# laboshinl/loam_velodyne

Hardware: AMD Instinct MI355X
Metric: sweeps/sec (64-ring, 1M-pt map): feature extraction + odometry + scan-to-map registration (higher is better)
Workload: dtype f32

## Files before the change

### include/loamx.h

```cpp
#ifndef LOAMX_H
#define LOAMX_H

#include <stddef.h>
#include <stdint.h>

#ifdef __cplusplus
extern "C" {
#endif

#define LOAMX_OK 0
#define LOAMX_SKIPPED 1
#define LOAMX_E_INVALID (-1)
#define LOAMX_E_CAPACITY (-2)
#define LOAMX_E_HIP (-3)
#define LOAMX_E_NOGPU (-4)
#define LOAMX_E_UNSUPPORTED (-5)

typedef struct loamx_cloud {
  void* data;
  uint32_t count;
  uint32_t stride;
  uint32_t intensity_offset;
  uint32_t reserved;
} loamx_cloud;

const char* loamx_last_error(void);
int loamx_device_count(void);
#define LOAMX_ABI_VERSION 6
int loamx_abi_version(void);
const char* loamx_build_info(void);
void* loamx_host_alloc(size_t bytes);
void loamx_host_free(void* p);

typedef struct loamx_scanreg loamx_scanreg;

typedef struct loamx_scanreg_config {
  float scan_period;
  int n_feature_regions;
  int curvature_region;
  int max_corner_sharp;
  int max_surface_flat;
  float less_flat_filter_size;
  float surface_curvature_threshold;
  int device;
  int max_corner_less_sharp;
  int imu_history_size;
} loamx_scanreg_config;

void loamx_scanreg_default_config(loamx_scanreg_config* cfg);
loamx_scanreg* loamx_scanreg_create(const loamx_scanreg_config* cfg);
void loamx_scanreg_destroy(loamx_scanreg* h);
int loamx_scanreg_configure(loamx_scanreg* h, const loamx_scanreg_config* cfg);
int loamx_scanreg_process(loamx_scanreg* h, const loamx_cloud* cloud, const uint32_t* ring_size, uint32_t n_rings,
                          loamx_cloud* sharp, loamx_cloud* less_sharp, loamx_cloud* flat, loamx_cloud* less_flat);

typedef struct loamx_multiscan_mapper {
  float lower_bound_deg;
  float upper_bound_deg;
  uint32_t n_scan_rings;
} loamx_multiscan_mapper;
int loamx_multiscan_mapper_preset(const char* sensor , loamx_multiscan_mapper* out);
int loamx_scanreg_process_raw(loamx_scanreg* h, const loamx_multiscan_mapper* mapper, const void* raw_xyz, uint32_t count,
                              uint32_t stride, loamx_cloud* full, uint32_t* ring_size, loamx_cloud* sharp, loamx_cloud* less_sharp,
                              loamx_cloud* flat, loamx_cloud* less_flat);

int loamx_scanreg_update_imu(loamx_scanreg* h, double stamp_sec, float roll, float pitch, float yaw, const float acc_xyz[3]);
int loamx_scanreg_set_time(loamx_scanreg* h, double scan_time_sec);
int loamx_scanreg_get_imu_trans(loamx_scanreg* h, float imu_trans[12]);

typedef struct loamx_odom loamx_odom;

typedef struct loamx_odom_config {
  float scan_period;
  int max_iterations;
  float delta_t_abort;
  float delta_r_abort;
  int device;
} loamx_odom_config;

void loamx_odom_default_config(loamx_odom_config* cfg);
loamx_odom* loamx_odom_create(const loamx_odom_config* cfg);
void loamx_odom_destroy(loamx_odom* h);
int loamx_odom_update_imu(loamx_odom* h, const float imu_trans[12]);
int loamx_odom_process(loamx_odom* h, const loamx_cloud* sharp, const loamx_cloud* less_sharp, const loamx_cloud* flat,
                       const loamx_cloud* less_flat);
int loamx_odom_get_transform(loamx_odom* h, float transform[6]);
int loamx_odom_get_transform_sum(loamx_odom* h, float transform_sum[6]);
int loamx_odom_set_transform(loamx_odom* h, const float transform[6]);
int loamx_odom_set_transform_sum(loamx_odom* h, const float transform_sum[6]);
int loamx_odom_get_last_clouds(loamx_odom* h, loamx_cloud* last_corner, loamx_cloud* last_surf);
int loamx_odom_transform_to_end(loamx_odom* h, loamx_cloud* cloud);
int loamx_odom_get_stats(loamx_odom* h, int stats[4]);

int loamx_scanreg_process_linked(loamx_scanreg* h, const loamx_cloud* cloud, const uint32_t* ring_size, uint32_t n_rings);
int loamx_odom_process_linked(loamx_odom* h, loamx_scanreg* sr);
int loamx_odom_link_wait(loamx_odom* h);

typedef struct loamx_map loamx_map;

typedef struct loamx_map_config {
  float scan_period;
  int max_iterations;
  float delta_t_abort;
  float delta_r_abort;
  float corner_filter_size;
  float surf_filter_size;
  float map_filter_size;
  int device;
} loamx_map_config;

void loamx_map_default_config(loamx_map_config* cfg);
loamx_map* loamx_map_create(const loamx_map_config* cfg);
void loamx_map_destroy(loamx_map* h);
int loamx_map_update_odometry(loamx_map* h, const float transform_sum[6]);
int loamx_map_process(loamx_map* h, const loamx_cloud* corner_last, const loamx_cloud* surf_last, loamx_cloud* full_res);
int loamx_map_process_linked(loamx_map* h, loamx_odom* od, loamx_cloud* full_res_registered);
int loamx_map_get_speculation(loamx_map* h, uint64_t counts[2]);
int loamx_map_insert(loamx_map* h, const loamx_cloud* corner_last, const loamx_cloud* surf_last, const float pose6[6]);
int loamx_map_get_transform(loamx_map* h, int which, float transform[6]);
int loamx_map_set_transform(loamx_map* h, int which, const float transform[6]);
int loamx_map_update_imu(loamx_map* h, double stamp_sec, float roll, float pitch);
int loamx_map_set_time(loamx_map* h, double laser_odometry_time_sec);
int loamx_map_has_fresh_map(loamx_map* h);
int loamx_map_get_surround(loamx_map* h, loamx_cloud* out);
int loamx_map_load_cubes(loamx_map* h, const loamx_cloud* corner, const loamx_cloud* surf);
int loamx_map_get_cubes(loamx_map* h, int which, loamx_cloud* out);
int loamx_map_save_snapshot(loamx_map* h, const char* path);
int loamx_map_load_snapshot(loamx_map* h, const char* path);
int loamx_map_set_timing(loamx_map* h, int on);
int loamx_map_get_timing(loamx_map* h, float ms[4], uint64_t counts[4]);
int loamx_map_get_stats(loamx_map* h, int stats[8]);

typedef struct loamx_tm loamx_tm;
loamx_tm* loamx_tm_create(void);
void loamx_tm_destroy(loamx_tm* h);
int loamx_tm_update_odometry(loamx_tm* h, const float transform_sum[6]);
int loamx_tm_update_mapping_transform(loamx_tm* h, const float aft_mapped[6], const float bef_mapped[6]);
int loamx_tm_associate_to_map(loamx_tm* h);
int loamx_tm_get_mapped(loamx_tm* h, float transform_mapped[6]);
int loamx_wire_pose_to_quat(const float rot_xyz[3], double quat_xyzw[4]);
int loamx_wire_quat_to_pose(const double quat_xyzw[4], float rot_xyz[3]);

typedef struct loamx_batch loamx_batch;

loamx_batch* loamx_batch_create(const loamx_map_config* cfg, uint32_t max_sweeps);
void loamx_batch_destroy(loamx_batch* h);
int loamx_batch_set_frozen(loamx_batch* h, const loamx_cloud* corner_map, const loamx_cloud* surf_map);
int loamx_batch_set_frozen_device(loamx_batch* h, const void* d_corner_xyzi, uint32_t n_corner, const void* d_surf_xyzi,
                                  uint32_t n_surf);
int loamx_batch_stage_frozen_device(loamx_batch* h, const void* d_corner_xyzi, uint32_t n_corner, const void* d_surf_xyzi,
                                    uint32_t n_surf, void* wait_event );
int loamx_batch_stage_frozen(loamx_batch* h, const loamx_cloud* corner_map, const loamx_cloud* surf_map);
int loamx_batch_swap_frozen(loamx_batch* h);
int loamx_batch_upload(loamx_batch* h, uint32_t n_sweeps, const loamx_cloud* corner_last, const loamx_cloud* surf_last,
                       const loamx_cloud* full_res, const float* guess6);
int loamx_batch_run(loamx_batch* h);
int loamx_batch_run_async(loamx_batch* h);
int loamx_batch_sync(loamx_batch* h);
int loamx_batch_download(loamx_batch* h, float* poses6, int* stats4);
int loamx_batch_download_full_res(loamx_batch* h, uint32_t sweep, loamx_cloud* out);
int loamx_batch_set_timing(loamx_batch* h, int on);
int loamx_batch_get_timing(loamx_batch* h, float ms[4], uint64_t counts[4]);
void* loamx_batch_stream(loamx_batch* h);
int loamx_batch_knn_probe(loamx_batch* h, int which, const float* queries_xyz, uint32_t n, uint32_t* idx5, float* d2_5);
int loamx_batch_qr6_probe(loamx_batch* h, const float* ata, const float* atb, uint32_t n, float* x_coop, float* x_scalar);
int loamx_batch_xrec_stress(loamx_batch* h, uint32_t pairs, uint32_t rounds, uint64_t out4[4]);
int loamx_batch_download_ds(loamx_batch* h, uint32_t sweep, loamx_cloud* corner_ds, loamx_cloud* surf_ds);

typedef struct loamx_pipeline loamx_pipeline;

loamx_pipeline* loamx_pipeline_create(const loamx_scanreg_config* fcfg, const loamx_odom_config* ocfg,
                                      const loamx_map_config* mcfg, uint32_t n_streams);
void loamx_pipeline_destroy(loamx_pipeline* h);
int loamx_pipeline_set_frozen(loamx_pipeline* h, const loamx_cloud* corner_map, const loamx_cloud* surf_map);
int loamx_pipeline_set_frozen_device(loamx_pipeline* h, const void* d_corner_xyzi, uint32_t n_corner, const void* d_surf_xyzi,
                                     uint32_t n_surf);
int loamx_pipeline_stage_frozen_device(loamx_pipeline* h, const void* d_corner_xyzi, uint32_t n_corner, const void* d_surf_xyzi,
                                       uint32_t n_surf, void* wait_event);
int loamx_pipeline_stage_frozen(loamx_pipeline* h, const loamx_cloud* corner_map, const loamx_cloud* surf_map);
int loamx_pipeline_swap_frozen(loamx_pipeline* h);
int loamx_pipeline_set_state(loamx_pipeline* h, uint32_t stream, const float* transform, const float* transform_sum,
                             const float* bef_mapped, const float* aft_mapped);
int loamx_pipeline_upload(loamx_pipeline* h, uint32_t n_steps, const loamx_cloud* clouds, const uint32_t* const* ring_size,
                          const uint32_t* n_rings);
int loamx_pipeline_stage_step(loamx_pipeline* h, uint32_t step, const loamx_cloud* clouds, const uint32_t* const* ring_size,
                              const uint32_t* n_rings);
int loamx_pipeline_stage_step_raw(loamx_pipeline* h, uint32_t step, const void* const* raw_xyz, const uint32_t* counts, uint32_t stride,
                                  const loamx_multiscan_mapper* mapper, const double* scan_time_sec);
int loamx_pipeline_update_imu(loamx_pipeline* h, uint32_t stream, double stamp_sec, float roll, float pitch, float yaw, const float acc_xyz[3]);
int loamx_pipeline_enable_async_downloads(loamx_pipeline* h);
int loamx_pipeline_download_step_async(loamx_pipeline* h, loamx_cloud* out, uint32_t n_out);
int loamx_pipeline_wait_downloads(loamx_pipeline* h);
int loamx_pipeline_download_counts(loamx_pipeline* h, uint64_t counts[2]);
int loamx_pipeline_step(loamx_pipeline* h, uint32_t step);
int loamx_pipeline_get(loamx_pipeline* h, uint32_t stream, float* transform, float* transform_sum, float* aft_mapped,
                       int* stats8);
int loamx_pipeline_download_full_res(loamx_pipeline* h, uint32_t slot, loamx_cloud* out);
int loamx_pipeline_download_last_clouds(loamx_pipeline* h, uint32_t stream, loamx_cloud* last_corner, loamx_cloud* last_surf);
int loamx_pipeline_set_lookahead(loamx_pipeline* h, int on);
int loamx_pipeline_lookahead_depth(loamx_pipeline* h);
int loamx_pipeline_drain_lookahead(loamx_pipeline* h, int* last_odometry_step);
int loamx_pipeline_set_timing(loamx_pipeline* h, int on);
int loamx_pipeline_get_timing(loamx_pipeline* h, float stage_ms[4], float reg_ms[4], uint64_t counts[4]);
int loamx_pipeline_get_odom_launch_timing(loamx_pipeline* h, double ms4[4], uint64_t counts7[7]);
void* loamx_pipeline_stream(loamx_pipeline* h);

typedef struct loamx_dist loamx_dist;
#define LOAMX_DIST_ID_BYTES 128
int loamx_dist_get_unique_id(unsigned char id[LOAMX_DIST_ID_BYTES]);
loamx_dist* loamx_dist_create(const unsigned char id[LOAMX_DIST_ID_BYTES], int rank, int world_size, int device);
void loamx_dist_destroy(loamx_dist* h);
int loamx_dist_rank(const loamx_dist* h);
int loamx_dist_world_size(const loamx_dist* h);
int loamx_dist_shard(const loamx_dist* h, uint32_t batch, uint32_t* begin, uint32_t* end);
int loamx_dist_broadcast_map(loamx_dist* h, void* d_corner_xyzi, uint32_t n_corner, void* d_surf_xyzi, uint32_t n_surf, int root,
                             void* wait_event, void** done_event);
int loamx_dist_allgather_results(loamx_dist* h, const float* poses6, const int* iters_flags2, uint32_t n_local, float* poses6_all,
                                 int* iters_flags2_all, uint32_t* counts_all);
int loamx_dist_allgather_results_cap(loamx_dist* h, const float* poses6, const int* iters_flags2, uint32_t n_local, float* poses6_all,
                                     int* iters_flags2_all, uint32_t capacity_records, uint32_t* counts_all);
int loamx_dist_allgather_counts(loamx_dist* h, uint32_t n_local, uint32_t* counts_all);
int loamx_dist_comm_count(loamx_dist* h);
#define LOAMX_DIST_RECORD_FLOATS 8
int loamx_dist_shard_of(int rank, int world_size, uint32_t batch, uint32_t* begin, uint32_t* end);
int loamx_dist_pack_results(const float* poses6, const int* iters_flags2, uint32_t n_local, uint32_t n_pad, float* send8);
int loamx_dist_unpack_results(const float* recv8, const uint32_t* counts, int world_size, uint32_t n_pad, float* poses6_all,
                              int* iters_flags2_all);
int loamx_dist_pack_clouds(uint32_t n_streams, const loamx_cloud* corner, const loamx_cloud* surf, const float* poses6, uint32_t* words,
                           uint64_t capacity_words, uint64_t* n_words);
int loamx_dist_unpack_clouds_header(const uint32_t* words, uint64_t n_words, uint32_t* n_streams, uint32_t* n_corner, uint32_t* n_surf,
                                    uint32_t capacity_streams);
int loamx_dist_unpack_clouds_stream(const uint32_t* words, uint64_t n_words, uint32_t stream, float pose6[6], loamx_cloud* corner,
                                    loamx_cloud* surf);
int loamx_dist_gatherv(loamx_dist* h, const uint32_t* send_words, uint32_t n_words, int root, uint32_t* recv_words, uint64_t capacity_words,
                       uint32_t* counts_all);
int loamx_dist_barrier(loamx_dist* h);
void* loamx_dist_stream(loamx_dist* h);

#ifdef __cplusplus
}
#endif
#endif
```

### loam_velodyne_amd/csrc/api_odom.hip

```cpp
#include "api_handles.h"

using namespace loamx;

extern "C" {

void loamx_odom_default_config(loamx_odom_config* cfg) {
  if (!cfg) return;
  cfg->scan_period = 0.1f;
  cfg->max_iterations = 25;
  cfg->delta_t_abort = 0.1f;
  cfg->delta_r_abort = 0.1f;
  cfg->device = 0;
}

loamx_odom* loamx_odom_create(const loamx_odom_config* cfg) {
  loamx_odom* h = nullptr;
  guard([&]() {
    loamx_odom_config c;
    if (cfg) c = *cfg; else loamx_odom_default_config(&c);
    LX_REQUIRE(c.scan_period > 0.f, "scan_period must be positive");
    LX_REQUIRE(c.max_iterations >= 1 && c.max_iterations <= 255, "max_iterations must be in [1, 255]");
    LX_REQUIRE(c.delta_t_abort > 0.f && c.delta_r_abort > 0.f, "abort thresholds must be positive");
    h = new loamx_odom(c.device);
    h->od.params.scan_period = c.scan_period;
    h->od.params.max_iterations = c.max_iterations;
    h->od.params.delta_t_abort = c.delta_t_abort;
    h->od.params.delta_r_abort = c.delta_r_abort;
    return LOAMX_OK;
  });
  return h;
}
void loamx_odom_destroy(loamx_odom* h) { delete h; }

int loamx_odom_update_imu(loamx_odom* h, const float imu_trans[12]) {
  return guard([&]() {
    LX_REQUIRE(h && imu_trans, "NULL argument");
    h->od.update_imu(0, imu_trans);
    return LOAMX_OK;
  });
}
int loamx_odom_process(loamx_odom* h, const loamx_cloud* sharp, const loamx_cloud* less_sharp, const loamx_cloud* flat,
                       const loamx_cloud* less_flat) {
  return guard([&]() {
    LX_REQUIRE(h && sharp && less_sharp && flat && less_flat, "NULL argument");
    return h->od.process_host(sharp, less_sharp, flat, less_flat);
  });
}
int loamx_odom_process_linked(loamx_odom* h, loamx_scanreg* sr) {
  return guard([&]() {
    LX_REQUIRE(h && sr, "NULL argument");
    LX_REQUIRE(sr->fx.device() == h->od.device(), "linked handles must live on one device");
    const float4* p[4] = {nullptr, nullptr, nullptr, nullptr};
    uint32_t n[4] = {0, 0, 0, 0};
    const float4* full = sr->fx.d_cloud() + sr->fx.point_base(0);
    const uint32_t n_full = sr->fx.point_base(1) - sr->fx.point_base(0);
    if (sr->fx.split_results()) {
      sr->fx.device_results_front(0, p, n);
      return h->od.process_linked(p, n, full, n_full, [sr](const float4*& q, uint32_t& c) { sr->fx.device_results_lf(0, q, c); });
    }
    sr->fx.device_results(0, p, n);
    return h->od.process_linked(p, n, full, n_full);
  });
}
int loamx_odom_link_wait(loamx_odom* h) {
  return guard([&]() {
    LX_REQUIRE(h, "NULL handle");
    if (h->od.link_ready()) LX_HIP(hipEventSynchronize(h->od.link_ready()));
    return LOAMX_OK;
  });
}
int loamx_odom_get_transform(loamx_odom* h, float t[6]) {
  return guard([&]() { LX_REQUIRE(h && t, "NULL argument"); h->od.stream_state(0).transform.get(t); return LOAMX_OK; });
}
int loamx_odom_get_transform_sum(loamx_odom* h, float t[6]) {
  return guard([&]() { LX_REQUIRE(h && t, "NULL argument"); h->od.stream_state(0).transform_sum.get(t); return LOAMX_OK; });
}
int loamx_odom_set_transform(loamx_odom* h, const float t[6]) {
  return guard([&]() { LX_REQUIRE(h && t, "NULL argument"); h->od.stream_state(0).transform.set(t); return LOAMX_OK; });
}
int loamx_odom_set_transform_sum(loamx_odom* h, const float t[6]) {
  return guard([&]() { LX_REQUIRE(h && t, "NULL argument"); h->od.stream_state(0).transform_sum.set(t); return LOAMX_OK; });
}
int loamx_odom_get_last_clouds(loamx_odom* h, loamx_cloud* last_corner, loamx_cloud* last_surf) {
  return guard([&]() { LX_REQUIRE(h, "NULL handle"); return h->od.get_last_clouds(0, last_corner, last_surf); });
}
int loamx_odom_transform_to_end(loamx_odom* h, loamx_cloud* cloud) {
  return guard([&]() { LX_REQUIRE(h && cloud, "NULL argument"); return h->od.transform_to_end_host(0, cloud); });
}
int loamx_odom_get_stats(loamx_odom* h, int stats[4]) {
  return guard([&]() {
    LX_REQUIRE(h && stats, "NULL argument");
    OdomStats s = h->od.stream_state(0).stats;
    stats[0] = s.iterations; stats[1] = s.sel; stats[2] = s.frame; stats[3] = s.degenerate;
    return LOAMX_OK;
  });
}

}
```

### loam_velodyne_amd/csrc/odometry.hip

```cpp
#include "odometry.hpp"
#include "pinned_copy.hpp"
#include <chrono>
#include <cstring>
#include <type_traits>

namespace loamx {

constexpr int OD_THREADS = 256;
constexpr int OD_TR_STRIDE = OD_THREADS + 2;
constexpr int OD_PART_STRIDE = 2 * (2 * 16 * LX_NSUM) + 16;
[[maybe_unused]] constexpr int OD_PART_TS = 2 * (2 * 16 * LX_NSUM);

__device__ inline void sincos_f(float a, float& s, float& c) { sincosf(a, &s, &c); }

__device__ inline void transform_to_start(const float* T, float scan_period, const float4 pi, float& x, float& y, float& z) {
  const float s = (1.f / scan_period) * (pi.w - (float)(int)pi.w);
  x = pi.x - s * T[3];
  y = pi.y - s * T[4];
  z = pi.z - s * T[5];
  float sx, cx, sy, cy, sz, cz;
  sincos_f(-s * T[0], sx, cx);
  sincos_f(-s * T[1], sy, cy);
  sincos_f(-s * T[2], sz, cz);
  rot_z(x, y, cz, sz);
  rot_x(y, z, cx, sx);
  rot_y(x, z, cy, sy);
}

constexpr uint32_t OD_IDX_MASK = 0xffffffu;

__device__ inline float sqd(const float4& a, float x, float y, float z) {
  const float dx = a.x - x, dy = a.y - y, dz = a.z - z;
  return dx * dx + dy * dy + dz * dz;
}

__device__ inline void wave_argmin(float& d, int& j, int& order) {
#pragma unroll
  for (int off = 32; off > 0; off >>= 1) {
    const float od = __shfl_xor(d, off, 64);
    const int oj = __shfl_xor(j, off, 64);
    const int oo = __shfl_xor(order, off, 64);
    if (od < d || (od == d && oo < order)) { d = od; j = oj; order = oo; }
  }
}

__device__ inline int nn1_shells(const GridDesc& g, const float4* __restrict__ sorted, const uint32_t* __restrict__ cell_start, float qx,
                                 float qy, float qz, int lane, int L0, float best, int best_id) {
  float lbest = best;
  uint32_t lid = best_id >= 0 ? (uint32_t)best_id : 0xffffffffu;
  const float h = 1.0f / g.inv_h;
  const float fx = (qx - g.ox) * g.inv_h, fy = (qy - g.oy) * g.inv_h, fz = (qz - g.oz) * g.inv_h;
  const int cx = (int)floorf(fx), cy = (int)floorf(fy), cz = (int)floorf(fz);
  for (int L = L0;; L++) {
    const int side = 2 * L + 1, nrows = side * side;
    for (int r0 = 0; r0 < nrows; r0 += 64) {
      uint32_t b0 = 0, e0 = 0, b1 = 0, e1 = 0;
      {
        const int rr = r0 + lane;
        if (rr < nrows) {
          const int dz = rr / side - L, dy = rr % side - L;
          const int z = cz + dz, y = cy + dy;
          if (z >= 0 && z < g.nz && y >= 0 && y < g.ny) {
            const float gz = dz == 0 ? 0.f : (dz > 0 ? ((float)z - fz) : (fz - (float)(z + 1))) * h;
            const float gy = dy == 0 ? 0.f : (dy > 0 ? ((float)y - fy) : (fy - (float)(y + 1))) * h;
            const float gyz = (gy * gy + gz * gz) * 0.9999f;
            if (gyz < best) {
              const float rx = sqrtf(best - gyz) * g.inv_h * 1.0001f + 1e-3f;
              const int xlo = (int)floorf(fx - rx), xhi = (int)floorf(fx + rx);
              const bool face = (dz == -L || dz == L || dy == -L || dy == L);
              const uint32_t row = ((uint32_t)z * g.ny + y) * g.nx;
              int xa = cx - L, xb = face ? cx + L : cx - L;
              if (xa < xlo) xa = xlo;
              if (xb > xhi) xb = xhi;
              if (xa < 0) xa = 0;
              if (xb > g.nx - 1) xb = g.nx - 1;
              if (xa <= xb) { b0 = cell_start[row + xa]; e0 = cell_start[row + xb + 1]; }
              if (!face && L > 0) {
                const int xc = cx + L;
                if (xc >= xlo && xc <= xhi && xc >= 0 && xc <= g.nx - 1) { b1 = cell_start[row + xc]; e1 = cell_start[row + xc + 1]; }
              }
            }
          }
        }
      }
      unsigned long long todo = __ballot(e0 > b0 || e1 > b1);
      while (todo) {
        const int src = __builtin_ctzll(todo);
        todo &= todo - 1;
        const uint32_t rb0 = __shfl(b0, src, 64), re0 = __shfl(e0, src, 64), rb1 = __shfl(b1, src, 64), re1 = __shfl(e1, src, 64);
        for (int part = 0; part < 2; part++) {
          const uint32_t beg = part ? rb1 : rb0, end = part ? re1 : re0;
          for (uint32_t k = beg + lane; k < end; k += 64) {
            const float4 p = sorted[k];
            const float dx = qx - p.x, dy2 = qy - p.y, dz2 = qz - p.z;
            const float d2 = dx * dx + dy2 * dy2 + dz2 * dz2;
            const uint32_t id = __float_as_uint(p.w) & OD_IDX_MASK;
            if (d2 < lbest || (d2 == lbest && lid != 0xffffffffu && id < lid)) { lbest = d2; lid = id; }
          }
        }
      }
    }
    float d = lbest;
    int j = (int)lid, o_ = (int)lid;
    if (lid == 0xffffffffu) { j = -1; o_ = 0x7fffffff; }
    wave_argmin(d, j, o_);
    if (j >= 0 && d < 25.0f) { best = d; best_id = j; }
    const float cover = (float)L * h;
    if (best <= cover * cover) break;
    if (cover * cover >= 25.0f) break;
  }
  return best_id;
}
#ifdef OD_CORR_WAVES
#define OD_CORR_ATTR __attribute__((amdgpu_waves_per_eu(OD_CORR_WAVES, OD_CORR_WAVES)))
#else
#define OD_CORR_ATTR
#endif
struct Block27 {
  uint32_t E[9], O[9];
  uint32_t total;
};
__device__ inline void block27_build(const GridDesc& g, const uint32_t* __restrict__ cell_start, float qx, float qy, float qz, int lane, Block27& B) {
  const float fx = (qx - g.ox) * g.inv_h, fy = (qy - g.oy) * g.inv_h, fz = (qz - g.oz) * g.inv_h;
  const int cx = (int)floorf(fx), cy = (int)floorf(fy), cz = (int)floorf(fz);
  uint32_t v = 0u;
  {
    const int r = lane >> 1, z = cz + r / 3 - 1, y = cy + r % 3 - 1;
    if (lane < 18 && z >= 0 && z < g.nz && y >= 0 && y < g.ny) {
      int xx = (lane & 1) ? cx + 2 : cx - 1;
      xx = xx < 0 ? 0 : (xx > g.nx ? g.nx : xx);
      v = cell_start[((uint32_t)z * g.ny + y) * g.nx + xx];
    }
  }
  uint32_t acc = 0;
#pragma unroll
  for (int r = 0; r < 9; r++) {
    const uint32_t b = (uint32_t)__shfl((int)v, 2 * r, 64), e = (uint32_t)__shfl((int)v, 2 * r + 1, 64);
    B.O[r] = b - acc;
    acc += e > b ? e - b : 0u;
    B.E[r] = acc;
  }
  B.total = acc;
}
#ifndef OD_BLK_CACHE
#define OD_BLK_CACHE 2
#endif
struct Block27First { float4 p[OD_BLK_CACHE > 0 ? OD_BLK_CACHE : 1]; };
template <bool LOAD_FIRST, class F>
__device__ inline void block27_scan(const Block27& B, const float4* __restrict__ sorted, int lane, Block27First& first, F&& visit) {
  for (uint32_t c0 = (uint32_t)lane; c0 < B.total; c0 += 4 * 64) {
    const bool first_trip = c0 == (uint32_t)lane;
    uint32_t pos[4];
    float4 p[4];
#pragma unroll
    for (int u = 0; u < 4; u++) {
      const uint32_t cc = c0 + 64u * u;
      uint32_t o = B.O[8];
#pragma unroll
      for (int k = 7; k >= 0; k--) o = cc < B.E[k] ? B.O[k] : o;
      pos[u] = cc < B.total ? cc + o : B.O[0];
    }
    if (LOAD_FIRST || !first_trip) {
#pragma unroll
      for (int u = 0; u < 4; u++) p[u] = sorted[pos[u]];
      if (LOAD_FIRST && first_trip) {
#pragma unroll
        for (int u = 0; u < OD_BLK_CACHE; u++) first.p[u] = p[u];
      }
    } else {
#pragma unroll
      for (int u = OD_BLK_CACHE; u < 4; u++) p[u] = sorted[pos[u]];
#pragma unroll
      for (int u = 0; u < OD_BLK_CACHE; u++) p[u] = first.p[u];
    }
#pragma unroll
    for (int u = 0; u < 4; u++) visit(p[u], (c0 + 64u * u) < B.total);
  }
}
__device__ inline int nn1_block(const GridDesc& g, const Block27& B, const float4* __restrict__ sorted, const uint32_t* __restrict__ cell_start,
                                float qx, float qy, float qz, int lane, uint32_t& w_out, Block27First& first) {
  float lbest = 25.0f;
  uint32_t lw = 0xffffffffu;
  block27_scan<true>(B, sorted, lane, first, [&](const float4& p, bool valid) {
    const float dx = qx - p.x, dy2 = qy - p.y, dz2 = qz - p.z;
    const float d2 = dx * dx + dy2 * dy2 + dz2 * dz2;
    const uint32_t w = __float_as_uint(p.w);
    if (valid && (d2 < lbest || (d2 == lbest && lw != 0xffffffffu && (w & OD_IDX_MASK) < (lw & OD_IDX_MASK)))) { lbest = d2; lw = w; }
  });
  float d = lbest;
  int j = lw == 0xffffffffu ? -1 : (int)(lw & OD_IDX_MASK), o_ = lw == 0xffffffffu ? 0x7fffffff : (int)(lw & OD_IDX_MASK);
  int ring = (int)(lw >> 24);
  {
#pragma unroll
    for (int off = 32; off > 0; off >>= 1) {
      const float od = __shfl_xor(d, off, 64);
      const int oj = __shfl_xor(j, off, 64), oo = __shfl_xor(o_, off, 64), orr = __shfl_xor(ring, off, 64);
      if (od < d || (od == d && oo < o_)) { d = od; j = oj; o_ = oo; ring = orr; }
    }
  }
  const float h = 1.0f / g.inv_h;
  if (j >= 0 && d < 25.0f && d <= h * h) { w_out = ((uint32_t)ring << 24) | (uint32_t)j; return j; }
  const int id = nn1_shells(g, sorted, cell_start, qx, qy, qz, lane, 2, (j >= 0 && d < 25.0f) ? d : 25.0f, (j >= 0 && d < 25.0f) ? j : -1);
  w_out = id == j ? (((uint32_t)ring << 24) | (uint32_t)j) : (0xff000000u | (uint32_t)(id < 0 ? 0 : id));
  return id;
}

constexpr int OD_RF_N = 320;
#ifdef LOAMX_PROF_CORR
__device__ unsigned long long g_corr_ts[3][16];
#define OC_TS(k) do { if (blockIdx.y == 0 && lane == 0 && ts_slot >= 0) g_corr_ts[ts_slot][k] = wall_clock64(); } while (0)
#else
#define OC_TS(k) do { } while (0)
#endif
__global__ __launch_bounds__(256) OD_CORR_ATTR void k_odom_corr_grid(OdomProblem* __restrict__ probs, OdomParams P, uint32_t* __restrict__ patch_dst, uint4 patch) {
  if (patch_dst && blockIdx.x == 0 && blockIdx.y == 0 && threadIdx.x == 0) { patch_dst[0] = patch.x; patch_dst[1] = patch.y; patch_dst[2] = patch.z; }
  OdomProblem& pb = probs[blockIdx.y];
  if (pb.done) return;
  const int lane = threadIdx.x & 63, wid = threadIdx.x >> 6;
  const int nSharp = (int)pb.n_sharp, nFlat = (int)pb.n_flat;
  int f;
  {
    const int x = (int)(blockIdx.x % 8), j = (int)(blockIdx.x / 8);
    const int sS = (int)((long long)x * nSharp / 8), nS = (int)((long long)(x + 1) * nSharp / 8) - sS;
    const int sF = (int)((long long)x * nFlat / 8), nF = (int)((long long)(x + 1) * nFlat / 8) - sF;
    const int fl = 4 * j + wid;
    if (fl >= nS + nF) return;
    f = fl < nS ? sS + fl : nSharp + sF + (fl - nS);
  }
#ifdef LOAMX_PROF_CORR
  const int ts_slot = f == nSharp / 2 ? 0 : f == nSharp + nFlat / 2 ? 1 : f == nSharp + nFlat - 1 ? 2 : -1;
#endif
  OC_TS(0);
  float T[6];
#pragma unroll
  for (int k = 0; k < 6; k++) T[k] = pb.transform[k];
  const bool corner = f < nSharp;
  const float4 pi = corner ? pb.sharp[f] : pb.flat[f - nSharp];
  const uint32_t* __restrict__ tbl = corner ? pb.rf_corner : pb.rf_surf;
  const int e0 = max((int)pi.w - 8, 0);
  uint32_t tv = 0u, unordered_epoch = 0u;
  if (tbl) {
    if (e0 + lane < OD_RF_N - 1) tv = tbl[e0 + lane];
    unordered_epoch = tbl[OD_RF_N - 1];
  }
  float x, y, z;
  transform_to_start(T, P.scan_period, pi, x, y, z);
  const GridDescB gd = corner ? *pb.lc_desc : *pb.ls_desc;
  const float4* __restrict__ sorted = pb.sorted;
  const uint32_t* __restrict__ cell_start = pb.cell_table + gd.cell_base;
  OC_TS(1);
  Block27 B;
  block27_build(gd.g, cell_start, x, y, z, lane, B);
  OC_TS(2);
  uint32_t wbest = 0u;
  Block27First first;
  const int closest = nn1_block(gd.g, B, sorted, cell_start, x, y, z, lane, wbest, first);
  OC_TS(3);
  if (closest < 0) {
    if (lane == 0) { pb.ind[5 * f] = -1; pb.ind[5 * f + 1] = -1; pb.ind[5 * f + 2] = -1; }
    return;
  }
  const float4* last = corner ? pb.last_corner : pb.last_surf;
  const int nLast = corner ? (int)pb.n_last_corner : (int)pb.n_last_surf;
  const int nCur = corner ? nSharp : nFlat;
  const int bound = nCur < nLast ? nCur : nLast;
  const int cscan = (wbest >> 24) != 255u ? (int)(wbest >> 24) : (int)last[closest].w;
  float d2 = 25.f, d3 = 25.f;
  int j2 = -1, j3 = -1, o2 = 0x7fffffff, o3 = 0x7fffffff;
  auto better = [](float d, int order, float dbest, int obest) { return d < dbest || (d == dbest && obest != 0x7fffffff && order < obest); };

  bool via_block = false;
  if (tbl && unordered_epoch != pb.rf_epoch && cscan < 255 && B.total > 0u) {
    const unsigned long long valid = __ballot(e0 + lane < OD_RF_N - 1 && (tv >> 24) == pb.rf_epoch);
    auto first_from = [&](int ring) -> int {
      const int k = ring - e0;
      if (k >= 64) return nLast;
      const unsigned long long m = k <= 0 ? valid : (valid >> k) << k;
      if (!m) return nLast;
      const int w = (int)((uint32_t)__shfl((int)tv, __builtin_ctzll(m), 64) & OD_IDX_MASK);
      return w < nLast ? w : nLast;
    };
    if (cscan - 2 >= e0 || e0 == 0) {
      const int wlo = min(first_from(cscan - 2), closest);
      const int whi = closest + 1 < bound ? max(min(bound, first_from(cscan + 3)), closest + 1) : closest + 1;
      const unsigned walk = (unsigned)(closest - wlo) + (unsigned)(whi - (closest + 1));
      via_block = walk > B.total + 128u;
    }
  }
  OC_TS(4);
  if (via_block) {
    block27_scan<false>(B, sorted, lane, first, [&](const float4& p, bool ok) {
      const uint32_t w = __float_as_uint(p.w);
      const int j = (int)(w & OD_IDX_MASK), ring = (int)(w >> 24);
      const float d = sqd(p, x, y, z);
      if (ok && j > closest && j < bound && ring <= cscan + 2) {
        const int order = j - (closest + 1);
        if (corner) {
          if (ring > cscan && better(d, order, d2, o2)) { d2 = d; j2 = j; o2 = order; }
        } else {
          if (ring <= cscan) { if (better(d, order, d2, o2)) { d2 = d; j2 = j; o2 = order; } }
          else { if (better(d, order, d3, o3)) { d3 = d; j3 = j; o3 = order; } }
        }
      } else if (ok && j < closest && ring >= cscan - 2) {
        const int order = 0x40000000 + (closest - 1 - j);
        if (corner) {
          if (ring < cscan && better(d, order, d2, o2)) { d2 = d; j2 = j; o2 = order; }
        } else {
          if (ring >= cscan) { if (better(d, order, d2, o2)) { d2 = d; j2 = j; o2 = order; } }
          else { if (better(d, order, d3, o3)) { d3 = d; j3 = j; o3 = order; } }
        }
      }
    });
    wave_argmin(d2, j2, o2);
    if (!corner) wave_argmin(d3, j3, o3);
    const float h = 1.0f / gd.g.inv_h, h2 = h * h;
    via_block = d2 < h2 && (corner || d3 < h2);
    if (!via_block) { d2 = d3 = 25.f; j2 = j3 = -1; o2 = o3 = 0x7fffffff; }
  }
  OC_TS(5);
  if (!via_block) {
    int baseF = closest + 1, baseB = closest - 1;
    bool stopF = baseF >= bound, stopB = baseB < 0;
    while (!stopF || !stopB) {
      float4 qf[4], qb[4];
      if (!stopF) {
#pragma unroll
        for (int u = 0; u < 4; u++) {
          const int j = baseF + 64 * u + lane;
          qf[u] = j < bound ? last[j] : make_float4(0.f, 0.f, 0.f, 0.f);
        }
      }
      if (!stopB) {
#pragma unroll
        for (int u = 0; u < 4; u++) {
          const int j = baseB - 64 * u - lane;
          qb[u] = j >= 0 ? last[j] : make_float4(0.f, 0.f, 0.f, 0.f);
        }
      }
      if (!stopF) {
        bool stop = false;
#pragma unroll
        for (int u = 0; u < 4; u++) {
          if (stop) continue;
          const int j = baseF + 64 * u + lane;
          const bool in = j < bound;
          const int ring = (int)qf[u].w;
          const bool brk = in && ((double)ring > (double)cscan + 2.5);
          const unsigned long long mb = __ballot(brk);
          const int fb = mb ? __builtin_ctzll(mb) : 64;
          if (in && lane < fb) {
            const float d = sqd(qf[u], x, y, z);
            const int order = j - (closest + 1);
            if (corner) {
              if (ring > cscan && better(d, order, d2, o2)) { d2 = d; j2 = j; o2 = order; }
            } else {
              if (ring <= cscan) { if (better(d, order, d2, o2)) { d2 = d; j2 = j; o2 = order; } }
              else { if (better(d, order, d3, o3)) { d3 = d; j3 = j; o3 = order; } }
            }
          }
          if (mb) stop = true;
        }
        baseF += 256;
        stopF = stop || baseF >= bound;
      }
      if (!stopB) {
        bool stop = false;
#pragma unroll
        for (int u = 0; u < 4; u++) {
          if (stop) continue;
          const int j = baseB - 64 * u - lane;
          const bool in = j >= 0;
          const int ring = (int)qb[u].w;
          const bool brk = in && ((double)ring < (double)cscan - 2.5);
          const unsigned long long mb = __ballot(brk);
          const int fb = mb ? __builtin_ctzll(mb) : 64;
          if (in && lane < fb) {
            const float d = sqd(qb[u], x, y, z);
            const int order = 0x40000000 + (closest - 1 - j);
            if (corner) {
              if (ring < cscan && better(d, order, d2, o2)) { d2 = d; j2 = j; o2 = order; }
            } else {
              if (ring >= cscan) { if (better(d, order, d2, o2)) { d2 = d; j2 = j; o2 = order; } }
              else { if (better(d, order, d3, o3)) { d3 = d; j3 = j; o3 = order; } }
            }
          }
          if (mb) stop = true;
        }
        baseB -= 256;
        stopB = stop || baseB < 0;
      }
    }
    wave_argmin(d2, j2, o2);
    if (!corner) wave_argmin(d3, j3, o3);
  }
  OC_TS(6);
  if (lane == 0) {
    pb.ind[5 * f] = closest;
    pb.ind[5 * f + 1] = j2;
    pb.ind[5 * f + 2] = corner ? -1 : j3;
  }
#ifdef LOAMX_PROF_CORR
  if (blockIdx.y == 0 && lane == 0 && ts_slot >= 0) {
    g_corr_ts[ts_slot][7] = wall_clock64();
    g_corr_ts[ts_slot][8] = (unsigned long long)B.total; g_corr_ts[ts_slot][9] = (unsigned long long)via_block;
    g_corr_ts[ts_slot][10] = (unsigned long long)closest; g_corr_ts[ts_slot][11] = (unsigned long long)cscan;
  }
#endif
}

#ifdef LOAMX_PROF_LM
#define LM_TS(k) do { if (blockIdx.x == 0 && blockIdx.y == 0 && tid == 0 && iter == it_begin + 1) pb.part[OD_PART_TS + (k)] = (double)wall_clock64(); } while (0)
#else
#define LM_TS(k) do { } while (0)
#endif
#ifndef OD_LM_WAVES
#define OD_LM_WAVES 3
#endif
#ifndef OD_LM_WAVES_MIN
#define OD_LM_WAVES_MIN 3
#endif
#define OD_LM_ATTR __attribute__((amdgpu_waves_per_eu(OD_LM_WAVES_MIN, OD_LM_WAVES)))
#pragma clang diagnostic push
#pragma clang diagnostic ignored "-Wpass-failed"
template <int OD_FPT>
__global__ __launch_bounds__(OD_THREADS) OD_LM_ATTR void k_odom_lm(OdomProblem* __restrict__ probs, OdomParams P, int iter0, int n_iters) {
  OdomProblem& pb = probs[blockIdx.y];
  if (pb.done) return;
  const unsigned NB = gridDim.x;
  const int tid = threadIdx.x;
  const int nSharp = (int)pb.n_sharp, nFlat = (int)pb.n_flat, nFeat = nSharp + nFlat;
  __shared__ float T[6];
  __shared__ float trig[6];
  __shared__ double red[8][LX_NSUM];
  using TrT = typename std::conditional<OD_FPT == 1, float, double>::type;
  __shared__ TrT tr[LX_NSUM * OD_TR_STRIDE];
  __shared__ int sh_done, sh_degen, sh_abort;
  __shared__ float matP[36];
  __shared__ float ws[216];
  __shared__ double parts[16 * LX_NSUM];
  __shared__ float AtA[36], AtB[6];
  if (tid < 6) {
    T[tid] = pb.transform[tid];
    const double ang = (double)pb.transform[tid >> 1];
    trig[tid] = (float)((tid & 1) ? cos(ang) : sin(ang));
  }
  const unsigned xtag = pb.xchg_epoch << 8;
  if (tid == 0) { sh_done = 0; sh_abort = 0; sh_degen = pb.stats.degenerate; }
  if (tid < 36) matP[tid] = pb.matP[tid];
  __syncthreads();

  float4 fpo[OD_FPT], ft1[OD_FPT], ft2[OD_FPT], ft3[OD_FPT];
  bool fvalid[OD_FPT], fcorner[OD_FPT];
#pragma unroll
  for (int u = 0; u < OD_FPT; u++) {
    const int f = (u * (int)NB + (int)blockIdx.x) * OD_THREADS + tid;
    fvalid[u] = false;
    fcorner[u] = f < nSharp;
    fpo[u] = ft1[u] = ft2[u] = ft3[u] = make_float4(0.f, 0.f, 0.f, 0.f);
    if (f < nFeat) {
      const int i1 = pb.ind[5 * f], i2 = pb.ind[5 * f + 1], i3 = pb.ind[5 * f + 2];
      if (fcorner[u] ? (i2 >= 0) : (i2 >= 0 && i3 >= 0)) {
        fvalid[u] = true;
        fpo[u] = fcorner[u] ? pb.sharp[f] : pb.flat[f - nSharp];
        const float4* last = fcorner[u] ? pb.last_corner : pb.last_surf;
        ft1[u] = last[i1];
        ft2[u] = last[i2];
        if (!fcorner[u]) ft3[u] = last[i3];
      }
    }
  }

  const int it_begin = iter0, it_end = iter0 + n_iters;
  for (int iter = it_begin; iter < it_end; iter++) {
    LM_TS(0);
    LM_TS(1);
    double v[OD_FPT == 1 ? 1 : LX_NSUM];
    float a1[6] = {0.f, 0.f, 0.f, 0.f, 0.f, 0.f}, bb1 = 0.f;
    bool sel1 = false;
#pragma unroll
    for (int k = 0; k < (OD_FPT == 1 ? 1 : LX_NSUM); k++) v[k] = 0.0;
#pragma unroll
    for (int u = 0; u < OD_FPT; u++) {
      if (!fvalid[u]) continue;
      const bool corner = fcorner[u];
      const float4 po = fpo[u];
      float cx = 0.f, cy = 0.f, cz = 0.f, ci = 0.f;
      bool sel = false;
      {
        float x0, y0, z0;
        transform_to_start(T, P.scan_period, po, x0, y0, z0);
        if (corner) {
          const float4 t1 = ft1[u], t2 = ft2[u];
          const float x1 = t1.x, y1 = t1.y, z1 = t1.z, x2 = t2.x, y2 = t2.y, z2 = t2.z;
          const float a012 = sqrtf(((x0 - x1) * (y0 - y2) - (x0 - x2) * (y0 - y1)) * ((x0 - x1) * (y0 - y2) - (x0 - x2) * (y0 - y1)) +
                                   ((x0 - x1) * (z0 - z2) - (x0 - x2) * (z0 - z1)) * ((x0 - x1) * (z0 - z2) - (x0 - x2) * (z0 - z1)) +
                                   ((y0 - y1) * (z0 - z2) - (y0 - y2) * (z0 - z1)) * ((y0 - y1) * (z0 - z2) - (y0 - y2) * (z0 - z1)));
          const float l12 = sqrtf((x1 - x2) * (x1 - x2) + (y1 - y2) * (y1 - y2) + (z1 - z2) * (z1 - z2));
          const float la = ((y1 - y2) * ((x0 - x1) * (y0 - y2) - (x0 - x2) * (y0 - y1)) +
                            (z1 - z2) * ((x0 - x1) * (z0 - z2) - (x0 - x2) * (z0 - z1))) / a012 / l12;
          const float lb = -((x1 - x2) * ((x0 - x1) * (y0 - y2) - (x0 - x2) * (y0 - y1)) -
                             (z1 - z2) * ((y0 - y1) * (z0 - z2) - (y0 - y2) * (z0 - z1))) / a012 / l12;
          const float lc = -((x1 - x2) * ((x0 - x1) * (z0 - z2) - (x0 - x2) * (z0 - z1)) +
                             (y1 - y2) * ((y0 - y1) * (z0 - z2) - (y0 - y2) * (z0 - z1))) / a012 / l12;
          const float ld2 = a012 / l12;
          float s = 1;
          if (iter >= 5) s = 1 - 1.8f * fabsf(ld2);
          cx = s * la; cy = s * lb; cz = s * lc; ci = s * ld2;
          sel = ((double)s > 0.1) && (ld2 != 0);
        } else {
          const float4 t1 = ft1[u], t2 = ft2[u], t3 = ft3[u];
          float pa = (t2.y - t1.y) * (t3.z - t1.z) - (t3.y - t1.y) * (t2.z - t1.z);
          float pbb = (t2.z - t1.z) * (t3.x - t1.x) - (t3.z - t1.z) * (t2.x - t1.x);
          float pc = (t2.x - t1.x) * (t3.y - t1.y) - (t3.x - t1.x) * (t2.y - t1.y);
          float pd = -(pa * t1.x + pbb * t1.y + pc * t1.z);
          const float ps = sqrtf(pa * pa + pbb * pbb + pc * pc);
          pa /= ps; pbb /= ps; pc /= ps; pd /= ps;
          const float pd2 = pa * x0 + pbb * y0 + pc * z0 + pd;
          float s = 1;
          if (iter >= 5) s = 1 - 1.8f * fabsf(pd2) / sqrtf(sqrtf(x0 * x0 + y0 * y0 + z0 * z0));
          cx = s * pa; cy = s * pbb; cz = s * pc; ci = s * pd2;
          sel = ((double)s > 0.1) && (pd2 != 0);
        }
      }
      if (sel) {
        const float srx = trig[0], crx = trig[1], sry = trig[2], cry = trig[3], srz = trig[4], crz = trig[5];
        const float tx = T[3], ty = T[4], tz = T[5];
        const float px = po.x, py = po.y, pz = po.z;
        float a[6];
        a[0] = (-crx * sry * srz * px + crx * crz * sry * py + srx * sry * pz + tx * crx * sry * srz - ty * crx * crz * sry - tz * srx * sry) * cx +
               (srx * srz * px - crz * srx * py + crx * pz + ty * crz * srx - tz * crx - tx * srx * srz) * cy +
               (crx * cry * srz * px - crx * cry * crz * py - cry * srx * pz + tz * cry * srx + ty * crx * cry * crz - tx * crx * cry * srz) * cz;
        a[1] = ((-crz * sry - cry * srx * srz) * px + (cry * crz * srx - sry * srz) * py - crx * cry * pz + tx * (crz * sry + cry * srx * srz) +
                ty * (sry * srz - cry * crz * srx) + tz * crx * cry) * cx +
               ((cry * crz - srx * sry * srz) * px + (cry * srz + crz * srx * sry) * py - crx * sry * pz + tz * crx * sry -
                ty * (cry * srz + crz * srx * sry) - tx * (cry * crz - srx * sry * srz)) * cz;
        a[2] = ((-cry * srz - crz * srx * sry) * px + (cry * crz - srx * sry * srz) * py + tx * (cry * srz + crz * srx * sry) -
                ty * (cry * crz - srx * sry * srz)) * cx +
               (-crx * crz * px - crx * srz * py + ty * crx * srz + tx * crx * crz) * cy +
               ((cry * crz * srx - sry * srz) * px + (crz * sry + cry * srx * srz) * py + tx * (sry * srz - cry * crz * srx) -
                ty * (crz * sry + cry * srx * srz)) * cz;
        a[3] = -(cry * crz - srx * sry * srz) * cx + crx * srz * cy - (crz * sry + cry * srx * srz) * cz;
        a[4] = -(cry * srz + crz * srx * sry) * cx - crx * crz * cy - (sry * srz - cry * crz * srx) * cz;
        a[5] = crx * sry * cx - srx * cy - crx * cry * cz;
        const float bb = (float)(-0.05 * (double)ci);
        if (OD_FPT == 1) {
#pragma unroll
          for (int i = 0; i < 6; i++) a1[i] = a[i];
          bb1 = bb;
          sel1 = true;
        } else {
          int k = 0;
#pragma unroll
          for (int i = 0; i < 6; i++)
#pragma unroll
            for (int j = i; j < 6; j++) v[k++] += (double)(a[i] * a[j]);
#pragma unroll
          for (int i = 0; i < 6; i++) v[k++] += (double)(a[i] * bb);
          v[k] += 1.0;
        }
      }
    }
    LM_TS(2);
    if (OD_FPT == 1) {
      int k = 0;
#pragma unroll
      for (int i = 0; i < 6; i++)
#pragma unroll
        for (int j = i; j < 6; j++) tr[(k++) * OD_TR_STRIDE + tid] = (TrT)(a1[i] * a1[j]);
#pragma unroll
      for (int i = 0; i < 6; i++) tr[(k++) * OD_TR_STRIDE + tid] = (TrT)(a1[i] * bb1);
      tr[k * OD_TR_STRIDE + tid] = (TrT)(sel1 ? 1.f : 0.f);
    } else {
#pragma unroll
      for (int t = 0; t < LX_NSUM; t++) tr[t * OD_TR_STRIDE + tid] = (TrT)v[OD_FPT == 1 ? 0 : t];
    }
    __syncthreads();
    if (tid < 8 * LX_NSUM) {
      const int c = tid % LX_NSUM, g = tid / LX_NSUM;
      const TrT* col = tr + c * OD_TR_STRIDE + g;
      double x = 0.0;
#pragma unroll 8
      for (int j = 0; j < OD_THREADS / 8; j++) x += (double)col[8 * j];
      red[g][c] = x;
    }
    __syncthreads();
    LM_TS(3);
    double xs = 0.0;
    if (tid < LX_NSUM) {
#pragma unroll
      for (int w = 0; w < 8; w++) xs += red[w][tid];
      if (NB > 1) {
        xrec_store(reinterpret_cast<xrec_t*>(pb.part) + (((unsigned)iter & 1u) * 16u + blockIdx.x) * LX_NSUM + tid, xs, xtag | (unsigned)(iter + 1));
      }
    }
    if (NB > 1) {
      LM_TS(4);
      {
        const unsigned want = xtag | (unsigned)(iter + 1);
        const xrec_t* rec = reinterpret_cast<const xrec_t*>(pb.part) + ((unsigned)iter & 1u) * 16u * LX_NSUM;
        const unsigned long long t_in = wall_clock64();
        for (unsigned e = tid; e < NB * LX_NSUM; e += OD_THREADS) {
          unsigned spins = 0;
          xrec_t r = xrec_load(rec + e);
          while (r.x != want || r.w != want) {
            __builtin_amdgcn_s_sleep(1);
            if ((++spins & 1023u) == 0u && wall_clock64() - t_in > 200000000ull) { sh_abort = 1; break; }
            r = xrec_load(rec + e);
          }
          parts[e] = xrec_value(r);
        }
      }
      __syncthreads();
      if (sh_abort) {
        if (tid == 0) {
          pb.done = 1;
          if (pb.err_word) __hip_atomic_store(pb.err_word, 1u, __ATOMIC_RELAXED, __HIP_MEMORY_SCOPE_SYSTEM);
          if (pb.host_mirror) pb.host_mirror->done = -1;
        }
        return;
      }
      LM_TS(5);
    }
    if (tid < 64) {
      if (NB > 1 && tid < LX_NSUM) {
        xs = 0.0;
        for (unsigned b = 0; b < NB; b++) xs += parts[b * LX_NSUM + tid];
      }
      if (tid < 21) {
        int i = 0, rem = tid;
        while (rem >= 6 - i) { rem -= 6 - i; i++; }
        const int j = i + rem;
        AtA[i * 6 + j] = AtA[j * 6 + i] = (float)xs;
      } else if (tid < 27) {
        AtB[tid - 21] = (float)xs;
      }
      const int sel = (int)__hiloint2double(__builtin_amdgcn_readlane(__double2hiint(xs), 27), __builtin_amdgcn_readlane(__double2loint(xs), 27));
      __builtin_amdgcn_fence(__ATOMIC_SEQ_CST, "wavefront");
      LM_TS(7);
      float xl = 0.f;
      int done_now = 0;
      if (sel >= 10) {
        xl = qr_solve6_lanes(AtA, AtB);
        LM_TS(8);
        if (iter == 0) {
          if (tid == 0) sh_degen = degeneracy_projector(AtA, 10.f, matP, ws) ? 1 : 0;
          __builtin_amdgcn_fence(__ATOMIC_SEQ_CST, "wavefront");
          if (blockIdx.x == 0 && tid < 36) pb.matP[tid] = matP[tid];
        }
        const int degen = sh_degen;
        if (degen) {
          const int r = tid < 6 ? tid : 5;
          float acc = 0.f;
#pragma unroll
          for (int c = 0; c < 6; c++) acc += matP[r * 6 + c] * lane_get(xl, c);
          xl = acc;
        }
        float x6[6];
#pragma unroll
        for (int k = 0; k < 6; k++) x6[k] = lane_get(xl, k);
        const float d0 = (float)(x6[0] * 180.0 / M_PI), d1 = (float)(x6[1] * 180.0 / M_PI), d2 = (float)(x6[2] * 180.0 / M_PI);
        const float deltaR = (float)sqrt((double)d0 * d0 + (double)d1 * d1 + (double)d2 * d2);
        const float t0 = x6[3] * 100, t1 = x6[4] * 100, t2 = x6[5] * 100;
        const float deltaT = (float)sqrt((double)t0 * t0 + (double)t1 * t1 + (double)t2 * t2);
        done_now = (deltaR < P.delta_r_abort && deltaT < P.delta_t_abort) ? 1 : 0;
      }
      float tl = T[tid < 6 ? tid : 5];
      if (sel >= 10) {
        float nv = tl + xl;
        if (!isfinite(nv)) nv = 0.f;
        tl = nv;
      }
      const float a0 = lane_get(tl, 0), a1 = lane_get(tl, 1), a2 = lane_get(tl, 2);
      const double ang = (double)((tid >> 1) == 0 ? a0 : ((tid >> 1) == 1 ? a1 : a2));
      const float tg = (float)((tid & 1) ? cos(ang) : sin(ang));
      if (tid < 6) { T[tid] = tl; trig[tid] = tg; }
      if (tid == 0 && done_now) sh_done = 1;
      if (blockIdx.x == 0) {
        const bool final_now = done_now || iter == it_end - 1;
        if (tid < 6) pb.transform[tid] = tl;
        if (tid == 0) {
          pb.stats.iterations = iter + 1;
          pb.stats.sel = sel;
          if (iter == 0 && sel >= 10) pb.stats.degenerate = sh_degen;
          if (done_now) pb.done = 1;
        }
        if (final_now) {
          ToEndParams& Pe = *pb.te_out;
          if (tid < 6) {
            Pe.T[tid] = tl;
            if (tid & 1) Pe.cT[tid >> 1] = tg; else Pe.sT[tid >> 1] = tg;
          }
          if (pb.host_mirror) {
            OdomProblem* hm = pb.host_mirror;
            if (tid < 6) hm->transform[tid] = tl;
            if (tid == 0) {
              OdomStats stt;
              stt.iterations = iter + 1; stt.sel = sel; stt.frame = pb.stats.frame; stt.degenerate = sh_degen;
              hm->stats = stt;
              hm->done = done_now;
            }
          }
        }
      }
      LM_TS(9);
    }
    __syncthreads();
    if (sh_done) break;
  }
}

#pragma clang diagnostic pop

__device__ inline float4 to_end_point(float4 p, const ToEndParams& P) {
  const float s = (1.f / P.scan_period) * (p.w - (float)(int)p.w);
  float x = p.x - s * P.T[3], y = p.y - s * P.T[4], z = p.z - s * P.T[5];
  float sx, cx, sy, cy, sz, cz;
  sincos_f(-s * P.T[0], sx, cx);
  sincos_f(-s * P.T[1], sy, cy);
  sincos_f(-s * P.T[2], sz, cz);
  rot_z(x, y, cz, sz); rot_x(y, z, cx, sx); rot_y(x, z, cy, sy);
  rot_y(x, z, P.cT[1], P.sT[1]); rot_x(y, z, P.cT[0], P.sT[0]); rot_z(x, y, P.cT[2], P.sT[2]);
  x += P.T[3] - P.shift[0];
  y += P.T[4] - P.shift[1];
  z += P.T[5] - P.shift[2];
  rot_z(x, y, P.c_start[2], P.s_start[2]); rot_x(y, z, P.c_start[0], P.s_start[0]); rot_y(x, z, P.c_start[1], P.s_start[1]);
  rot_y(x, z, P.c_end[1], -P.s_end[1]); rot_x(y, z, P.c_end[0], -P.s_end[0]); rot_z(x, y, P.c_end[2], -P.s_end[2]);
  return make_float4(x, y, z, (float)(int)p.w);
}
__global__ __launch_bounds__(256) void k_transform_to_end_copy(float4* __restrict__ dst, const float4* __restrict__ src, uint32_t n, ToEndParams P) {
  const uint32_t i = blockIdx.x * blockDim.x + threadIdx.x;
  if (i >= n) return;
  dst[i] = to_end_point(src[i], P);
}
__global__ __launch_bounds__(256) void k_transform_to_end(float4* __restrict__ pts, uint32_t n, ToEndParams P) {
  const uint32_t i = blockIdx.x * blockDim.x + threadIdx.x;
  if (i >= n) return;
  pts[i] = to_end_point(pts[i], P);
}
__global__ void k_te_patch(const OdomProblem* __restrict__ probs, uint32_t na, ToEndParams* __restrict__ te) {
  const uint32_t a = blockIdx.x * blockDim.x + threadIdx.x;
  if (a >= na) return;
  const OdomProblem& pb = probs[a];
  ToEndParams& P = te[pb.stream_id];
  for (int k = 0; k < 6; k++) P.T[k] = pb.transform[k];
  for (int k = 0; k < 3; k++) {
    P.sT[k] = (float)sin((double)pb.transform[k]);
    P.cT[k] = (float)cos((double)pb.transform[k]);
  }
}

__global__ __launch_bounds__(256) void k_transform_to_end_batch(float4* __restrict__ pts, uint32_t n, const uint32_t* __restrict__ off,
                                                                uint32_t K, uint32_t ns, const ToEndParams* __restrict__ params,
                                                                const float4* __restrict__ src_c, const float4* __restrict__ src_s,
                                                                uint32_t n_corner_all, uint32_t* __restrict__ bounds,
                                                                uint32_t* __restrict__ ring_first, uint32_t rf_epoch) {
  const uint32_t i = blockIdx.x * blockDim.x + threadIdx.x;
  const bool active = i < n;
  uint32_t lo = 0;
  float4 q = make_float4(0.f, 0.f, 0.f, 0.f);
  if (active) {
    uint32_t hi = K;
    while (hi - lo > 1) {
      const uint32_t mid = (lo + hi) >> 1;
      if (off[mid] <= i) lo = mid; else hi = mid;
    }
    const ToEndParams P = params[lo % ns];
    if (src_c) {
      const float4 p = i < n_corner_all ? src_c[i] : src_s[i - n_corner_all];
      q = P.enabled ? to_end_point(p, P) : p;
      pts[i] = q;
    } else {
      q = pts[i];
      if (P.enabled) { q = to_end_point(q, P); pts[i] = q; }
    }
  }
  if (ring_first) {
    const int ring = (int)q.w;
    int prev = __shfl_up(ring, 1, 64);
    const uint32_t plo = (uint32_t)__shfl_up((int)lo, 1, 64);
    const bool first_in_cloud = active && i == off[lo];
    if (active && !first_in_cloud && (threadIdx.x & 63) == 0) {
      const uint32_t ip = i - 1;
      prev = (int)(src_c ? (ip < n_corner_all ? src_c[ip] : src_s[ip - n_corner_all]) : pts[ip]).w;
    } else if (active && plo != lo) {
      prev = -1;
    }
    if (active && ring >= 0 && ring < OD_RF_N - 1 && (first_in_cloud || prev != ring))
      ring_first[(size_t)lo * OD_RF_N + ring] = (rf_epoch << 24) | ((i - off[lo]) & OD_IDX_MASK);
    if (active && (ring < 0 || ring >= 255 || (i - off[lo]) > OD_IDX_MASK || (!first_in_cloud && prev > ring)))
      ring_first[(size_t)lo * OD_RF_N + OD_RF_N - 1] = rf_epoch;
  }
  if (bounds) cloud_bounds_update(bounds, active, lo, q.x, q.y, q.z);
}

__global__ __launch_bounds__(256) void k_to_end_gather(float4* __restrict__ dst, uint32_t n, const uint32_t* __restrict__ off, uint32_t K,
                                                       const float4* const* __restrict__ src, const uint32_t* __restrict__ sid,
                                                       const ToEndParams* __restrict__ params) {
  const uint32_t i = blockIdx.x * blockDim.x + threadIdx.x;
  if (i >= n) return;
  uint32_t lo = 0, hi = K;
  while (hi - lo > 1) {
    const uint32_t mid = (lo + hi) >> 1;
    if (off[mid] <= i) lo = mid; else hi = mid;
  }
  dst[i] = to_end_point(src[lo][i - off[lo]], params[sid[lo]]);
}

OdometryBatch::OdometryBatch(int device, uint32_t n_streams, hipStream_t shared_stream) : device_(device) {
  select_device(device);
  LX_REQUIRE(n_streams >= 1 && n_streams <= 1024, "n_streams must be in [1, 1024]");
  if (shared_stream) {
    st_ = shared_stream;
  } else {
    st_ = create_stream(env_priority("LOAMX_PRIO_ODOM", +1), 0, 0);
    own_stream_ = true;
  }
  for (uint32_t s = 0; s < n_streams; s++) streams_.push_back(new OdomStream());
  index_.cell_size = 2.1f;
  if (const char* e = diag_env("LOAMX_ODOM_CELL")) { const float v = (float)atof(e); if (v >= 0.25f && v <= 16.f) index_.cell_size = v; }
  index_.pack_ring = true;
  index_.init(st_);
  h_mirror_.reserve(n_streams);
  h_err_.reserve(16);
  rf_.reserve((size_t)2 * n_streams * OD_RF_N);
  LX_HIP(hipMemsetAsync(rf_.p, 0, sizeof(uint32_t) * 2 * n_streams * OD_RF_N, st_));
  memset(h_err_.p, 0, 16 * sizeof(uint32_t));
  part_.reserve((size_t)n_streams * OD_PART_STRIDE);
  LX_HIP(hipMemset(part_.p, 0, sizeof(double) * part_.cap));
  {
    auto up256 = [](size_t b) { return (b + 255) & ~(size_t)255; };
    const size_t o_te = up256(sizeof(OdomProblem) * n_streams), o_off = o_te + up256(sizeof(ToEndParams) * n_streams);
    up_bytes_ = o_off + up256(sizeof(uint32_t) * (2 * (size_t)n_streams + 2));
    up_dev_.reserve(up_bytes_);
    up_host_.reserve(up_bytes_);
    memset(up_host_.p, 0, up_bytes_);
    prob_.p = (OdomProblem*)up_dev_.p; h_prob_.p = (OdomProblem*)up_host_.p;
    te_.p = (ToEndParams*)(up_dev_.p + o_te); h_te_.p = (ToEndParams*)(up_host_.p + o_te);
    d_cur_off_.p = (uint32_t*)(up_dev_.p + o_off); h_off_pin_.p = (uint32_t*)(up_host_.p + o_off);
  }
  h_cur_off_.assign(2 * n_streams + 1, 0);
  h_last_off_.assign(2 * n_streams + 1, 0);
}

OdometryBatch::~OdometryBatch() {
  if (ev_tail_) (void)hipEventDestroy(ev_tail_);
  if (ev_up_) (void)hipEventDestroy(ev_up_);
  if (ev_pose_) (void)hipEventDestroy(ev_pose_);
  for (auto* p : streams_) delete p;
  for (auto& c : lt_) for (auto& e : c.ev) if (e) (void)hipEventDestroy(e);
  if (own_stream_ && st_) (void)hipStreamDestroy(st_);
}

void OdometryBatch::lt_resolve_() {
  for (auto& c : lt_) {
    if (!c.pending || !c.pairs) continue;
    if (hipEventQuery(c.ev[3 * (c.pairs - 1) + 2]) != hipSuccess) { (void)hipGetLastError(); continue; }
    for (int k = 0; k < c.pairs; k++) {
      float a = 0.f, b = 0.f;
      if (hipEventElapsedTime(&a, c.ev[3 * k], c.ev[3 * k + 1]) != hipSuccess || hipEventElapsedTime(&b, c.ev[3 * k + 1], c.ev[3 * k + 2]) != hipSuccess) { (void)hipGetLastError(); continue; }
      if (c.iters[k] > 0) {
        lt_tot_.corr_ms += a; lt_tot_.corr_launches++; lt_tot_.corr_features += c.feats[k];
        lt_tot_.lm_ms += b; lt_tot_.lm_launches++; lt_tot_.lm_iterations += (uint64_t)c.iters[k]; lt_tot_.lm_bytes += c.bytes[k];
      } else {
        lt_tot_.corr_noop_ms += a; lt_tot_.corr_noop_launches++;
        lt_tot_.lm_noop_ms += b; lt_tot_.lm_noop_launches++;
      }
    }
    c.pending = false;
  }
}
OdometryBatch::LaunchTotals OdometryBatch::launch_totals() {
  std::lock_guard<std::mutex> lk(lt_mu_);
  lt_resolve_();
  return lt_tot_;
}

void odom_set_imu(OdomStream& S, const float* t);
ToEndParams odom_to_end_params(const OdomStream& S, float scan_period, bool enabled);
void odom_integrate_pose(OdomStream& S);

void OdometryBatch::update_imu(uint32_t s, const float* t) { odom_set_imu(*streams_[s], t); }

ToEndParams OdometryBatch::to_end_params(uint32_t s, bool enabled) const { return odom_to_end_params(*streams_[s], params.scan_period, enabled); }

void OdometryBatch::to_end_device(uint32_t s, float4* pts, uint32_t n) {
  if (!n) return;
  hipLaunchKernelGGL(k_transform_to_end, dim3((n + 255) / 256), dim3(256), 0, st_, pts, n, to_end_params(s, true));
}

void odom_integrate_pose(OdomStream& S) {
  HAngle rx, ry, rz;
  accumulate_rotation(S.transform_sum.rot_x, S.transform_sum.rot_y, S.transform_sum.rot_z, -S.transform.rot_x,
                      HAngle((float)(-S.transform.rot_y.r * 1.05)), -S.transform.rot_z, rx, ry, rz);
  HVec3 v{S.transform.pos.x - S.imu_shift.x, S.transform.pos.y - S.imu_shift.y, (float)(S.transform.pos.z * 1.05 - S.imu_shift.z)};
  h_rot_zxy(v, rz, rx, ry);
  HVec3 trans{S.transform_sum.pos.x - v.x, S.transform_sum.pos.y - v.y, S.transform_sum.pos.z - v.z};
  plugin_imu_rotation(rx, ry, rz, S.imu_pitch_start, S.imu_yaw_start, S.imu_roll_start, S.imu_pitch_end, S.imu_yaw_end,
                      S.imu_roll_end, rx, ry, rz);
  S.transform_sum.rot_x = rx; S.transform_sum.rot_y = ry; S.transform_sum.rot_z = rz;
  S.transform_sum.pos = trans;
}
void odom_set_imu(OdomStream& S, const float* t) {
  S.imu_pitch_start = HAngle(t[0]); S.imu_yaw_start = HAngle(t[1]); S.imu_roll_start = HAngle(t[2]);
  S.imu_pitch_end = HAngle(t[3]); S.imu_yaw_end = HAngle(t[4]); S.imu_roll_end = HAngle(t[5]);
  S.imu_shift = {t[6], t[7], t[8]};
  S.imu_velo = {t[9], t[10], t[11]};
}
ToEndParams odom_to_end_params(const OdomStream& S, float scan_period, bool enabled) {
  ToEndParams P;
  S.transform.get(P.T);
  const HAngle* ta[3] = {&S.transform.rot_x, &S.transform.rot_y, &S.transform.rot_z};
  const HAngle* sa[3] = {&S.imu_pitch_start, &S.imu_yaw_start, &S.imu_roll_start};
  const HAngle* ea[3] = {&S.imu_pitch_end, &S.imu_yaw_end, &S.imu_roll_end};
  for (int k = 0; k < 3; k++) {
    P.sT[k] = ta[k]->s; P.cT[k] = ta[k]->c;
    P.s_start[k] = sa[k]->s; P.c_start[k] = sa[k]->c;
    P.s_end[k] = ea[k]->s; P.c_end[k] = ea[k]->c;
  }
  P.shift[0] = S.imu_shift.x; P.shift[1] = S.imu_shift.y; P.shift[2] = S.imu_shift.z;
  P.scan_period = scan_period;
  P.enabled = enabled ? 1 : 0;
  return P;
}

void OdometryBatch::process(const OdomInput* in, int* rc, bool defer_tail) {
  TraceRange trace_range("loamx:odometry");
  LX_HIP(hipSetDevice(device_));
  const uint32_t ns = n_streams(), K = 2 * ns;
  if (up_pending_) {
    LX_HIP(hipEventSynchronize(ev_up_));
    up_pending_ = false;
  }
  const bool late = ns == 1 && (bool)late_less_flat;
  std::vector<OdomInput> in_late;
  if (late) {
    in_late.assign(in, in + ns);
    in_late[0].less_flat = nullptr; in_late[0].n_less_flat = 0;
    in = in_late.data();
  }
  for (uint32_t s = 0; s < ns; s++) {
    h_cur_off_[s + 1] = h_cur_off_[s] + in[s].n_less_sharp;
    if (s > 0) LX_REQUIRE(in[s].less_sharp == in[s - 1].less_sharp + in[s - 1].n_less_sharp || in[s].n_less_sharp == 0 || in[s - 1].n_less_sharp == 0,
                          "less_sharp clouds of the streams must be contiguous");
  }
  for (uint32_t s = 0; s < ns; s++) h_cur_off_[ns + s + 1] = h_cur_off_[ns + s] + in[s].n_less_flat;
  const uint32_t n_corner_all = h_cur_off_[ns];
  uint32_t n_all = h_cur_off_[K];
  cur_.reserve((size_t)n_all + (late ? late_bound : 0u) + 1);
  bool contig_c = true, contig_s = true;
  for (uint32_t s = 1; s < ns; s++) {
    contig_c = contig_c && in[s].less_sharp == in[s - 1].less_sharp + in[s - 1].n_less_sharp;
    contig_s = contig_s && in[s].less_flat == in[s - 1].less_flat + in[s - 1].n_less_flat;
  }
  const bool fused_stage = contig_c && contig_s;
  const float4* src_c = fused_stage ? in[0].less_sharp : nullptr;
  const float4* src_s = fused_stage ? in[0].less_flat : nullptr;
  bool late_pending = late, patch_pending = false;
  auto resolve_late = [&]() {
    if (!late_pending) return;
    late_pending = false;
    const float4* p = nullptr;
    uint32_t n = 0;
    late_less_flat(p, n);
    LX_REQUIRE(n <= late_bound, "internal: the late less-flat cloud is larger than its announced bound");
    in_late[0].less_flat = p; in_late[0].n_less_flat = n;
    h_cur_off_[ns + 1] = h_cur_off_[ns] + n;
    n_all = h_cur_off_[K];
    src_s = p;
    patch_pending = true;
  };
  auto flush_patch = [&]() {
    if (!patch_pending) return;
    patch_pending = false;
    h_off_late_.reserve(K + 1);
    memcpy(h_off_late_.p, h_cur_off_.data(), sizeof(uint32_t) * (K + 1));
    LX_HIP(hipMemcpyAsync(d_cur_off_.p, h_off_late_.p, sizeof(uint32_t) * (K + 1), hipMemcpyHostToDevice, st_));
    LX_HIP(hipEventRecord(ev_up_, st_));
  };
  if (fused_stage) {
  } else if (contig_c) {
    if (n_corner_all) LX_HIP(hipMemcpyAsync(cur_.p, in[0].less_sharp, sizeof(float4) * n_corner_all, hipMemcpyDeviceToDevice, st_));
  } else {
    for (uint32_t s = 0; s < ns; s++)
      if (in[s].n_less_sharp) LX_HIP(hipMemcpyAsync(cur_.p + h_cur_off_[s], in[s].less_sharp, sizeof(float4) * in[s].n_less_sharp, hipMemcpyDeviceToDevice, st_));
  }
  if (fused_stage) {
  } else if (contig_s) {
    if (n_all > n_corner_all) LX_HIP(hipMemcpyAsync(cur_.p + n_corner_all, in[0].less_flat, sizeof(float4) * (n_all - n_corner_all), hipMemcpyDeviceToDevice, st_));
  } else {
    for (uint32_t s = 0; s < ns; s++)
      if (in[s].n_less_flat) LX_HIP(hipMemcpyAsync(cur_.p + h_cur_off_[ns + s], in[s].less_flat, sizeof(float4) * in[s].n_less_flat, hipMemcpyDeviceToDevice, st_));
  }

  xchg_epoch_ = xchg_epoch_ % 0xffffffu + 1u;
  std::vector<uint32_t> active;
  uint32_t max_feat = 0, max_sharp = 0, max_flat = 0, ind_total = 0;
  std::vector<uint32_t> ind_off(ns + 1, 0);
  for (uint32_t s = 0; s < ns; s++) ind_off[s + 1] = ind_off[s] + 5 * (in[s].n_sharp + in[s].n_flat) + 5;
  ind_total = ind_off[ns];
  ind_.reserve(ind_total + 8);
  for (uint32_t s = 0; s < ns; s++) {
    OdomStream& S = *streams_[s];
    const OdomInput& I = in[s];
    if (!S.inited) {
      S.transform_sum.rot_x = HAngle(S.transform_sum.rot_x.r + S.imu_pitch_start.r);
      S.transform_sum.rot_z = HAngle(S.transform_sum.rot_z.r + S.imu_roll_start.r);
      rc[s] = LOAMX_SKIPPED;
      continue;
    }
    rc[s] = LOAMX_OK;
    S.frame++;
    S.transform.pos.x -= S.imu_velo.x * params.scan_period;
    S.transform.pos.y -= S.imu_velo.y * params.scan_period;
    S.transform.pos.z -= S.imu_velo.z * params.scan_period;
    S.stats = {0, 0, (int)S.frame, 0};
    if (S.n_last_corner > 10 && S.n_last_surf > 100) {
      OdomProblem& pb = h_prob_.p[active.size()];
      pb.sharp = I.sharp; pb.n_sharp = I.n_sharp;
      pb.flat = I.flat; pb.n_flat = I.n_flat;
      pb.last_corner = last_.p + h_last_off_[s]; pb.n_last_corner = S.n_last_corner;
      pb.last_surf = last_.p + h_last_off_[ns + s]; pb.n_last_surf = S.n_last_surf;
      pb.sorted = index_.sorted();
      pb.cell_table = index_.cell_table();
      pb.lc_desc = index_.desc(s);
      pb.ls_desc = index_.desc(ns + s);
      pb.ind = ind_.p + ind_off[s];
      S.transform.get(pb.transform);
      pb.stats = {0, 0, 0, 0};
      pb.done = 0;
      pb.ticket = 0;
      pb.xchg_epoch = xchg_epoch_;
      pb.stream_id = (int)s;
      pb.host_mirror = h_mirror_.p + active.size();
      pb.te_out = te_.p + s;
      pb.part = part_.p + (size_t)active.size() * OD_PART_STRIDE;
      pb.err_word = h_err_.p;
      pb.rf_corner = rf_.p + (size_t)s * OD_RF_N;
      pb.rf_surf = rf_.p + (size_t)(ns + s) * OD_RF_N;
      pb.rf_epoch = rf_epoch_;
      max_feat = std::max(max_feat, I.n_sharp + I.n_flat);
      max_sharp = std::max(max_sharp, I.n_sharp);
      max_flat = std::max(max_flat, I.n_flat);
      active.push_back(s);
    }
  }
  const uint32_t na = (uint32_t)active.size();
  if (max_feat > 32 * OD_THREADS) throw Error(LOAMX_E_CAPACITY, "more than 8192 sharp+flat features in one sweep");
  for (uint32_t s = 0; s < ns; s++) h_te_.p[s] = to_end_params(s, rc[s] == LOAMX_OK);
  memcpy(h_off_pin_.p, h_cur_off_.data(), sizeof(uint32_t) * (K + 1));
  LX_HIP(hipMemcpyAsync(up_dev_.p, up_host_.p, up_bytes_, hipMemcpyHostToDevice, st_));
  index_.prepare(K);
  const bool index_prepared = true;
  if (!ev_up_) LX_HIP(hipEventCreateWithFlags(&ev_up_, hipEventDisableTiming));
  LX_HIP(hipEventRecord(ev_up_, st_));
  up_pending_ = true;
  LtCall* lt = nullptr;
  if (launch_timing_.load(std::memory_order_relaxed) && na && max_feat) {
    std::lock_guard<std::mutex> lk(lt_mu_);
    lt_resolve_();
    LtCall& c = lt_[lt_next_ % LT_RING];
    if (!c.pending) { lt = &c; lt_next_++; c.pairs = 0; }
  }
  if (na) {
    if (max_feat) {
      const int pair_mode = [] { const char* e = getenv("LOAMX_ODOM_PAIRS"); return !e ? 1 : !strcmp(e, "all") ? 0 : !strcmp(e, "exact") ? 2 : !strcmp(e, "lag2") ? 3 : 1; }();
      const int maxp = (params.max_iterations + 4) / 5;
      for (uint32_t a = 0; a < na; a++) { h_mirror_.p[a].done = 0; h_mirror_.p[a].stats.iterations = 0; }
      auto enqueue_corr = [&](int k) {
        const int lk = lt && k < LT_MAXP ? k : -1;
        if (lk >= 0) {
          for (int e = 0; e < 3; e++) if (!lt->ev[3 * lk + e]) LX_HIP(hipEventCreate(&lt->ev[3 * lk + e]));
          LX_HIP(hipEventRecord(lt->ev[3 * lk], st_));
        }
        uint32_t* pd = nullptr;
        uint4 pv = make_uint4(0u, 0u, 0u, 0u);
        if (patch_pending) { patch_pending = false; pd = d_cur_off_.p; pv = make_uint4(h_cur_off_[0], h_cur_off_[1], h_cur_off_[2], 0u); }
        hipLaunchKernelGGL(k_odom_corr_grid, dim3(8 * (((max_sharp + 7) / 8 + (max_flat + 7) / 8 + 3) / 4), na), dim3(256), 0, st_, prob_.p, params, pd, pv);
        if (lk >= 0) LX_HIP(hipEventRecord(lt->ev[3 * lk + 1], st_));
      };
      auto enqueue_lm = [&](int k) {
        const int it0 = 5 * k;
        const int nit = std::min(5, params.max_iterations - it0);
        const int lk = lt && k < LT_MAXP ? k : -1;
#ifdef OD_LM_HALF_WGS
        const uint32_t nb = std::min<uint32_t>(16u, std::max<uint32_t>(1u, (max_feat + 2 * OD_THREADS - 1) / (2 * OD_THREADS)));
#else
        const uint32_t nb = std::min<uint32_t>(16u, (max_feat + OD_THREADS - 1) / OD_THREADS);
#endif
        const bool two = max_feat > nb * OD_THREADS;
        if (!lm_slots_[two]) {
          int per_cu = 0;
          if (two) LX_HIP(hipOccupancyMaxActiveBlocksPerMultiprocessor(&per_cu, k_odom_lm<2>, OD_THREADS, 0));
          else LX_HIP(hipOccupancyMaxActiveBlocksPerMultiprocessor(&per_cu, k_odom_lm<1>, OD_THREADS, 0));
          hipDeviceProp_t prop;
          LX_HIP(hipGetDeviceProperties(&prop, device_));
          lm_slots_[two] = (uint32_t)std::max(per_cu, 1) * (uint32_t)std::max(prop.multiProcessorCount, 1);
        }
        const uint32_t chunk = std::max<uint32_t>(1u, (lm_slots_[two] / 2) / nb);
        for (uint32_t a0 = 0; a0 < na; a0 += chunk) {
          const uint32_t nc = std::min(chunk, na - a0);
          if (two) hipLaunchKernelGGL(k_odom_lm<2>, dim3(nb, nc), dim3(OD_THREADS), 0, st_, prob_.p + a0, params, it0, nit);
          else hipLaunchKernelGGL(k_odom_lm<1>, dim3(nb, nc), dim3(OD_THREADS), 0, st_, prob_.p + a0, params, it0, nit);
        }
        if (lk >= 0) { LX_HIP(hipEventRecord(lt->ev[3 * lk + 2], st_)); lt->pairs = lk + 1; }
      };
      auto enqueue_pair = [&](int it0) { enqueue_corr(it0 / 5); enqueue_lm(it0 / 5); };
      const volatile OdomProblem* hm = h_mirror_.p;
      auto settled = [&](int k) {
        const int want = std::min(5 * (k + 1), params.max_iterations);
        for (uint32_t a = 0; a < na; a++) if (hm[a].done == 0 && hm[a].stats.iterations < want) return false;
        return true;
      };
      auto converged = [&]() {
        for (uint32_t a = 0; a < na; a++) if (hm[a].done == 0 && hm[a].stats.iterations < params.max_iterations) return false;
        return true;
      };
      auto wait_settled = [&](int k) {
        const auto t_in = std::chrono::steady_clock::now();
        for (unsigned spins = 0; !settled(k);) {
          if ((++spins & 255u) == 0u && std::chrono::steady_clock::now() - t_in > std::chrono::milliseconds(20)) return false;
          __builtin_ia32_pause();
        }
        return true;
      };
      int enq = 0;
      if (pair_mode == 1) {
        enqueue_corr(0);
        enqueue_lm(0);
        enq = 1;
        if (maxp > 1) enqueue_corr(1);
        resolve_late();
        while (enq < maxp) {
          if (!wait_settled(enq - 1)) {
            enqueue_lm(enq);
            for (enq++; enq < maxp; enq++) enqueue_pair(5 * enq);
            break;
          }
          if (converged()) break;
          enqueue_lm(enq);
          enq++;
          if (enq < maxp) enqueue_corr(enq);
        }
      } else {
      const int first = pair_mode == 0 ? maxp : std::min(maxp, pair_mode == 2 ? std::max(1, pred_pairs_) : 2);
      for (; enq < first; enq++) enqueue_pair(5 * enq);
      resolve_late();
      bool blind = false;
      while (enq < maxp) {
        const int watch = pair_mode == 2 ? enq - 1 : enq - 2;
        if (!blind && watch >= 0) {
          if (!wait_settled(watch)) blind = true;
          if (!blind && converged()) break;
        }
        enqueue_pair(5 * enq);
        enq++;
      }
      }
      pairs_enqueued_ += (uint64_t)enq;
      pair_calls_++;
    }
    if (!max_feat) LX_HIP(hipMemcpyAsync(h_mirror_.p, prob_.p, sizeof(OdomProblem) * na, hipMemcpyDeviceToHost, st_));
    if (!ev_pose_) LX_HIP(hipEventCreateWithFlags(&ev_pose_, hipEventDisableTiming));
    LX_HIP(hipEventRecord(ev_pose_, st_));
    if (!max_feat) hipLaunchKernelGGL(k_te_patch, dim3((na + 63) / 64), dim3(64), 0, st_, prob_.p, na, te_.p);
  }
  static const bool fuse_bounds = !(diag_env("LOAMX_BB_FUSED") && atoi(diag_env("LOAMX_BB_FUSED")) == 0);
  resolve_late();
  flush_patch();
  if (n_all)
  {
    if (++rf_epoch_ > 255u) rf_epoch_ = 1u;
    hipLaunchKernelGGL(k_transform_to_end_batch, dim3((n_all + 255) / 256), dim3(256), 0, st_, cur_.p, n_all, d_cur_off_.p, K, ns, te_.p, src_c,
                       src_s, n_corner_all, fuse_bounds ? index_.d_bounds() : nullptr, rf_.p, rf_epoch_);
  }
  {
    float4* p = cur_.p; size_t c = cur_.cap;
    DevBuf<float4>& oldest = older_[keep_ - 2];
    cur_.p = oldest.p; cur_.cap = oldest.cap;
    for (int k = keep_ - 2; k > 0; k--) { older_[k].p = older_[k - 1].p; older_[k].cap = older_[k - 1].cap; }
    older_[0].p = last_.p; older_[0].cap = last_.cap;
    last_.p = p; last_.cap = c;
  }
  h_last_off_ = h_cur_off_;
  index_.build(last_.p, h_last_off_.data(), K, d_cur_off_.p, index_prepared, fuse_bounds && n_all > 0);
  if (!ev_tail_) LX_HIP(hipEventCreateWithFlags(&ev_tail_, hipEventDisableTiming));
  LX_HIP(hipEventRecord(ev_tail_, st_));
  tail_pending_ = true;
  if (na) {
    wait_event(ev_pose_);
    if (*(volatile uint32_t*)h_err_.p) {
      *h_err_.p = 0u;
      throw Error(LOAMX_E_HIP, "odometry: the exchange between a stream's k_odom_lm workgroups timed out (not all of them resident)");
    }
#ifdef LOAMX_PROF_CORR
    {
      unsigned long long ts[3][16];
      LX_HIP(hipMemcpyFromSymbol(ts, HIP_SYMBOL(g_corr_ts), sizeof(ts)));
      for (int q = 0; q < 3; q++)
        fprintf(stderr, "[corr ts %s, us since entry] feature+trig %.2f block table %.2f nn1 %.2f decision %.2f block windows %.2f walk %.2f end %.2f | block %llu pts, via block %llu, closest %lld cscan %lld\n",
                q == 0 ? "corner" : q == 1 ? "flat mid" : "flat last", (ts[q][1] - ts[q][0]) * 0.01, (ts[q][2] - ts[q][0]) * 0.01, (ts[q][3] - ts[q][0]) * 0.01,
                (ts[q][4] - ts[q][0]) * 0.01, (ts[q][5] - ts[q][0]) * 0.01, (ts[q][6] - ts[q][0]) * 0.01, (ts[q][7] - ts[q][0]) * 0.01, ts[q][8], ts[q][9],
                (long long)ts[q][10], (long long)ts[q][11]);
    }
#endif
#ifdef LOAMX_PROF_LM
    {
      double ts[16];
      LX_HIP(hipMemcpy(ts, part_.p + OD_PART_TS, sizeof(ts), hipMemcpyDeviceToHost));
      fprintf(stderr, "[lm ts, 10ns ticks]");
      for (int k = 1; k < 10; k++) fprintf(stderr, " %d:%+.0f", k, ts[k] - ts[0]);
      fprintf(stderr, "\n");
    }
#endif
    {
      int need = 1;
      for (uint32_t a = 0; a < na; a++) need = std::max(need, (h_mirror_.p[a].stats.iterations + 4) / 5);
      pred_pairs_ = need;
    }
    for (uint32_t a = 0; a < na; a++) {
      OdomStream& S = *streams_[active[a]];
      S.transform.set(h_mirror_.p[a].transform);
      S.stats.iterations = h_mirror_.p[a].stats.iterations;
      S.stats.sel = h_mirror_.p[a].stats.sel;
      S.stats.degenerate = h_mirror_.p[a].stats.degenerate;
    }
    if (lt) {
      std::lock_guard<std::mutex> lk(lt_mu_);
      for (int k = 0; k < lt->pairs; k++) {
        lt->iters[k] = 0; lt->bytes[k] = 0; lt->feats[k] = 0;
        for (uint32_t a = 0; a < na; a++) {
          const int it = h_mirror_.p[a].stats.iterations - 5 * k;
          if (it <= 0) continue;
          const uint64_t nf = (uint64_t)in[active[a]].n_sharp + in[active[a]].n_flat;
          lt->iters[k] = std::max(lt->iters[k], std::min(it, 5));
          lt->bytes[k] += 48ull * nf;
          lt->feats[k] += nf;
        }
      }
      lt->pending = true;
    }
  }
  for (uint32_t s = 0; s < ns; s++) {
    OdomStream& S = *streams_[s];
    if (rc[s] == LOAMX_OK) odom_integrate_pose(S);
    S.inited = true;
    S.n_last_corner = in[s].n_less_sharp;
    S.n_last_surf = in[s].n_less_flat;
  }
  if (!defer_tail) {
    LX_HIP(hipStreamSynchronize(st_));
    tail_pending_ = false;
  }
}

void OdometryBatch::to_end_gather(float4* dst, const uint32_t* h_off, const float4* const* src, const ToEndParams* seg_params, uint32_t K,
                                  hipStream_t stream) {
  const uint32_t n = h_off[K];
  if (!n) return;
  const uint32_t ns = K;
  const size_t bytes = sizeof(ToEndParams) * ns + sizeof(float4*) * K + sizeof(uint32_t) * (2 * (size_t)K + 2) + 64;
  h_gather_.reserve(bytes);
  d_gather_.reserve(bytes);
  char* h = h_gather_.p;
  ToEndParams* hp = (ToEndParams*)h;
  for (uint32_t s = 0; s < ns; s++) hp[s] = seg_params[s];
  const size_t o_src = (sizeof(ToEndParams) * ns + 15) & ~(size_t)15;
  const float4** hs = (const float4**)(h + o_src);
  for (uint32_t k = 0; k < K; k++) hs[k] = src[k];
  const size_t o_off = o_src + sizeof(float4*) * K;
  uint32_t* ho = (uint32_t*)(h + o_off);
  memcpy(ho, h_off, sizeof(uint32_t) * (K + 1));
  uint32_t* hsid = ho + K + 1;
  for (uint32_t k = 0; k < K; k++) hsid[k] = k;
  LX_HIP(hipMemcpyAsync(d_gather_.p, h, o_off + sizeof(uint32_t) * (2 * (size_t)K + 1), hipMemcpyHostToDevice, stream));
  char* d = d_gather_.p;
  hipLaunchKernelGGL(k_to_end_gather, dim3((n + 255) / 256), dim3(256), 0, stream, dst, n, (const uint32_t*)(d + o_off), K,
                     (const float4* const*)(d + o_src), (const uint32_t*)(d + o_off) + K + 1, (const ToEndParams*)d);
}

int OdometryBatch::process_host(const loamx_cloud* sharp, const loamx_cloud* less_sharp, const loamx_cloud* flat,
                                const loamx_cloud* less_flat) {
  LX_REQUIRE(n_streams() == 1, "process_host is the single-stream entry point");
  LX_HIP(hipSetDevice(device_));
  const loamx_cloud* cl[4] = {sharp, less_sharp, flat, less_flat};
  size_t off[5] = {0, 0, 0, 0, 0};
  for (int k = 0; k < 4; k++) {
    check_cloud(cl[k], false);
    off[k + 1] = off[k] + cl[k]->count;
  }
  h_stage_.reserve(off[4] + 1);
  up_[0].reserve(off[4] + 1);
  for (int k = 0; k < 4; k++) pack_cloud(cl[k], h_stage_.p + off[k]);
  if (!packed_all_finite(h_stage_.p, off[4])) throw Error(LOAMX_E_INVALID, "a feature cloud holds non-finite coordinates");
  fetch_from_pinned(up_[0].p, h_stage_.p, off[4], st_);
  OdomInput in{up_[0].p, sharp->count, up_[0].p + off[1], less_sharp->count, up_[0].p + off[2], flat->count, up_[0].p + off[3], less_flat->count};
  int rc = LOAMX_OK;
  last_dl_valid_ = false;
  process(&in, &rc, true);
  OdomStream& S = *streams_[0];
  const uint32_t n = S.n_last_corner + S.n_last_surf;
  h_last_dl_.reserve((size_t)n + 1);
  if (n) LX_HIP(hipMemcpyAsync(h_last_dl_.p, d_last_corner(0), sizeof(float4) * n, hipMemcpyDeviceToHost, st_));
  last_dl_valid_ = d_last_surf(0) == d_last_corner(0) + S.n_last_corner;
  return rc;
}

int OdometryBatch::process_linked(const float4* const feat[4], const uint32_t n_feat[4], const float4* d_full, uint32_t n_full,
                                  const std::function<void(const float4*&, uint32_t&)>& less_flat_late) {
  LX_REQUIRE(n_streams() == 1, "process_linked is a single-stream entry point");
  LX_HIP(hipSetDevice(device_));
  OdomInput in{feat[0], n_feat[0], feat[1], n_feat[1], feat[2], n_feat[2], feat[3], n_feat[3]};
  int rc = LOAMX_OK;
  last_dl_valid_ = false;
  link_valid_ = false;
  struct Late {
    OdometryBatch& o;
    ~Late() { o.late_less_flat = nullptr; o.late_bound = 0; }
  } late_guard{*this};
  if (less_flat_late) { late_less_flat = less_flat_late; late_bound = n_full; }
  process(&in, &rc, true);
  link_full_.reserve((size_t)n_full + 1);
  if (n_full)
    hipLaunchKernelGGL(k_transform_to_end_copy, dim3((n_full + 255) / 256), dim3(256), 0, st_, link_full_.p, d_full, n_full, to_end_params(0, true));
  n_link_full_ = n_full;
  if (!ev_link_) LX_HIP(hipEventCreateWithFlags(&ev_link_, hipEventDisableTiming));
  LX_HIP(hipEventRecord(ev_link_, st_));
  link_valid_ = true;
  return rc;
}

int OdometryBatch::get_last_clouds(uint32_t s, loamx_cloud* corner, loamx_cloud* surf) {
  LX_HIP(hipSetDevice(device_));
  OdomStream& S = *streams_[s];
  int rc = LOAMX_OK;
  if (corner) check_cloud(corner, false);
  if (surf) check_cloud(surf, false);
  if (last_dl_valid_ && s == 0) {
    LX_HIP(hipStreamSynchronize(st_));
    if (corner) {
      const int r = unpack_cloud(h_last_dl_.p, S.n_last_corner, corner);
      if (r != LOAMX_OK) rc = r;
    }
    if (surf) {
      const int r = unpack_cloud(h_last_dl_.p + S.n_last_corner, S.n_last_surf, surf);
      if (r != LOAMX_OK) rc = r;
    }
    return rc;
  }
  const uint32_t nc = corner ? S.n_last_corner : 0u, nsf = surf ? S.n_last_surf : 0u;
  h_stage_.reserve((size_t)nc + nsf + 1);
  if (nc) LX_HIP(hipMemcpyAsync(h_stage_.p, d_last_corner(s), sizeof(float4) * nc, hipMemcpyDeviceToHost, st_));
  if (nsf) LX_HIP(hipMemcpyAsync(h_stage_.p + nc, d_last_surf(s), sizeof(float4) * nsf, hipMemcpyDeviceToHost, st_));
  if (nc + nsf) LX_HIP(hipStreamSynchronize(st_));
  if (corner) {
    const int r = unpack_cloud(h_stage_.p, nc, corner);
    if (r != LOAMX_OK) rc = r;
  }
  if (surf) {
    const int r = unpack_cloud(h_stage_.p + nc, nsf, surf);
    if (r != LOAMX_OK) rc = r;
  }
  return rc;
}

int OdometryBatch::transform_to_end_host(uint32_t s, loamx_cloud* cloud) {
  LX_HIP(hipSetDevice(device_));
  check_cloud(cloud, false);
  const uint32_t n = cloud->count;
  h_stage_.reserve(n + 1);
  tmp_cloud_.reserve(n + 1);
  pack_cloud(cloud, h_stage_.p);
  fetch_from_pinned(tmp_cloud_.p, h_stage_.p, n, st_);
  to_end_device(s, tmp_cloud_.p, n);
  if (n) LX_HIP(hipMemcpyAsync(h_stage_.p, tmp_cloud_.p, sizeof(float4) * n, hipMemcpyDeviceToHost, st_));
  LX_HIP(hipStreamSynchronize(st_));
  return unpack_cloud(h_stage_.p, n, cloud);
}

}
```

### loam_velodyne_amd/csrc/odometry.hpp

```cpp
#pragma once
#include "common.h"
#include "host_math.h"
#include "registration.hpp"
#include <atomic>
#include <condition_variable>
#include <functional>
#include <mutex>
#include <thread>

namespace loamx {

struct OdomParams {
  float scan_period = 0.1f;
  int max_iterations = 25;
  float delta_t_abort = 0.1f, delta_r_abort = 0.1f;
};

struct OdomStats {
  int iterations, sel, frame, degenerate;
};

struct ToEndParams;

struct OdomProblem {
  const float4* sharp; uint32_t n_sharp;
  const float4* flat; uint32_t n_flat;
  const float4* last_corner; uint32_t n_last_corner;
  const float4* last_surf; uint32_t n_last_surf;
  const float4* sorted;
  const uint32_t* cell_table;
  const GridDescB* lc_desc;
  const GridDescB* ls_desc;
  int* ind;
  float transform[6];
  OdomStats stats;
  int done;
  float matP[36];
  int stream_id;
  ToEndParams* te_out;
  OdomProblem* host_mirror;
  unsigned ticket;
  unsigned xchg_epoch;
  double* part;
  const uint32_t* rf_corner;
  const uint32_t* rf_surf;
  uint32_t rf_epoch;
  uint32_t* err_word;
};

struct OdomInput {
  const float4* sharp; uint32_t n_sharp;
  const float4* less_sharp; uint32_t n_less_sharp;
  const float4* flat; uint32_t n_flat;
  const float4* less_flat; uint32_t n_less_flat;
};

struct ToEndParams {
  float T[6];
  float sT[3], cT[3];
  float shift[3];
  float s_start[3], c_start[3];
  float s_end[3], c_end[3];
  float scan_period;
  int enabled;
};

struct OdomStream {
  bool inited = false;
  long frame = 0;
  HTwist transform, transform_sum;
  HAngle imu_roll_start, imu_pitch_start, imu_yaw_start, imu_roll_end, imu_pitch_end, imu_yaw_end;
  HVec3 imu_shift, imu_velo;
  OdomStats stats = {0, 0, 0, 0};
  uint32_t n_last_corner = 0, n_last_surf = 0;
};

class OdometryBatch {
 public:
  OdometryBatch(int device, uint32_t n_streams, hipStream_t shared_stream = nullptr);
  ~OdometryBatch();
  OdomParams params;
  uint32_t n_streams() const { return (uint32_t)streams_.size(); }
  OdomStream& stream_state(uint32_t s) { return *streams_[s]; }
  hipStream_t stream() const { return st_; }
  void update_imu(uint32_t s, const float* t12);
  void process(const OdomInput* in, int* rc, bool defer_tail = false);
  hipEvent_t tail_event() const { return tail_pending_ ? ev_tail_ : nullptr; }
  void set_keep(int n) { keep_ = n < 2 ? 2 : (n > MAX_KEEP ? MAX_KEEP : n); }
  int process_host(const loamx_cloud* sharp, const loamx_cloud* less_sharp, const loamx_cloud* flat, const loamx_cloud* less_flat);
  int process_linked(const float4* const feat[4], const uint32_t n_feat[4], const float4* d_full, uint32_t n_full,
                     const std::function<void(const float4*&, uint32_t&)>& less_flat_late = nullptr);
  hipEvent_t link_ready() const { return ev_link_; }
  const float4* d_link_full() const { return link_full_.p; }
  uint32_t n_link_full() const { return n_link_full_; }
  bool link_valid() const { return link_valid_; }
  int device() const { return device_; }
  int get_last_clouds(uint32_t s, loamx_cloud* corner, loamx_cloud* surf);
  int transform_to_end_host(uint32_t s, loamx_cloud* cloud);
  void to_end_device(uint32_t s, float4* pts, uint32_t n);
  void to_end_gather(float4* dst, const uint32_t* h_off, const float4* const* src, const ToEndParams* seg_params, uint32_t K,
                     hipStream_t stream);
  ToEndParams to_end_params(uint32_t s, bool enabled) const;
  struct LaunchTotals {
    double lm_ms = 0, lm_noop_ms = 0, corr_ms = 0, corr_noop_ms = 0;
    uint64_t lm_launches = 0, lm_noop_launches = 0, lm_iterations = 0, corr_launches = 0, corr_noop_launches = 0;
    uint64_t lm_bytes = 0, corr_features = 0;
  };
  void set_launch_timing(bool on) { launch_timing_.store(on, std::memory_order_relaxed); }
  LaunchTotals launch_totals();
  const float4* d_last_corner(uint32_t s) const { return last_.p + h_last_off_[s]; }
  const float4* d_last_surf(uint32_t s) const { return last_.p + h_last_off_[n_streams() + s]; }

 private:
  int device_;
  hipStream_t st_ = nullptr;
  bool own_stream_ = false;
  std::vector<OdomStream*> streams_;
  DevBuf<float4> cur_, last_;
  static constexpr int MAX_KEEP = 16;
  DevBuf<float4> older_[MAX_KEEP - 1];
  int keep_ = 2;
  std::vector<uint32_t> h_cur_off_, h_last_off_;
  SubMapIndexBatch index_;
  DevBuf<int> ind_;
  DevBuf<double> part_;
  PinBuf<OdomProblem> h_mirror_;
  PinBuf<uint32_t> h_err_;
  DevBuf<uint32_t> rf_;
  uint32_t rf_epoch_ = 0;
  uint32_t xchg_epoch_ = 0;
  template <class T> struct View { T* p = nullptr; };
  DevBuf<char> up_dev_;
  PinBuf<char> up_host_;
  size_t up_bytes_ = 0;
  View<OdomProblem> prob_, h_prob_;
  View<ToEndParams> te_, h_te_;
  View<uint32_t> d_cur_off_, h_off_pin_;
  PinBuf<uint32_t> h_off_late_;
  std::function<void(const float4*&, uint32_t&)> late_less_flat;
  uint32_t late_bound = 0;
  PinBuf<float4> h_stage_;
  PinBuf<float4> h_last_dl_;
  bool last_dl_valid_ = false;
  DevBuf<float4> up_[4], tmp_cloud_, link_full_;
  uint32_t n_link_full_ = 0;
  bool link_valid_ = false;
  hipEvent_t ev_link_ = nullptr;
  int pred_pairs_ = 5;
  uint64_t pairs_enqueued_ = 0, pair_calls_ = 0;
  uint32_t lm_slots_[2] = {0, 0};
  hipEvent_t ev_tail_ = nullptr, ev_pose_ = nullptr, ev_up_ = nullptr;
  bool tail_pending_ = false, up_pending_ = false;
  PinBuf<char> h_gather_;
  DevBuf<char> d_gather_;
  static constexpr int LT_RING = 8, LT_MAXP = 8;
  struct LtCall {
    hipEvent_t ev[3 * LT_MAXP] = {};
    int pairs = 0;
    bool pending = false;
    int iters[LT_MAXP] = {};
    uint64_t bytes[LT_MAXP] = {}, feats[LT_MAXP] = {};
  };
  LtCall lt_[LT_RING];
  int lt_next_ = 0;
  std::atomic<bool> launch_timing_{false};
  std::mutex lt_mu_;
  LaunchTotals lt_tot_;
  void lt_resolve_();
};


}
```

### loam_velodyne_amd/loamx.py

```python
from __future__ import annotations

import ctypes as C
import os
import numpy as np

_HERE = os.path.dirname(os.path.abspath(__file__))
LIB_PATH = os.environ.get("LOAMX_LIB") or os.path.join(_HERE, "libloamx.so")

OK, SKIPPED, E_INVALID, E_CAPACITY, E_HIP, E_NOGPU, E_UNSUPPORTED = 0, 1, -1, -2, -3, -4, -5


class Cloud(C.Structure):
    _fields_ = [("data", C.c_void_p), ("count", C.c_uint32), ("stride", C.c_uint32),
                ("intensity_offset", C.c_uint32), ("reserved", C.c_uint32)]


class ScanRegConfig(C.Structure):
    _fields_ = [("scan_period", C.c_float), ("n_feature_regions", C.c_int), ("curvature_region", C.c_int),
                ("max_corner_sharp", C.c_int), ("max_surface_flat", C.c_int), ("less_flat_filter_size", C.c_float),
                ("surface_curvature_threshold", C.c_float), ("device", C.c_int), ("max_corner_less_sharp", C.c_int),
                ("imu_history_size", C.c_int)]


class OdomConfig(C.Structure):
    _fields_ = [("scan_period", C.c_float), ("max_iterations", C.c_int), ("delta_t_abort", C.c_float),
                ("delta_r_abort", C.c_float), ("device", C.c_int)]


class MapConfig(C.Structure):
    _fields_ = [("scan_period", C.c_float), ("max_iterations", C.c_int), ("delta_t_abort", C.c_float),
                ("delta_r_abort", C.c_float), ("corner_filter_size", C.c_float), ("surf_filter_size", C.c_float),
                ("map_filter_size", C.c_float), ("device", C.c_int)]


class LoamxError(RuntimeError):
    def __init__(self, code, msg):
        super().__init__(f"loamx error {code}: {msg}")
        self.code = code


_lib = None


def lib():
    global _lib
    if _lib is None:
        if not os.path.exists(LIB_PATH):
            raise FileNotFoundError(f"{LIB_PATH} not built: run `python -c 'import __graft_entry__ as g; g.build()'` "
                                    "(no CPU fallback exists)")
        L = C.CDLL(LIB_PATH)
        L.loamx_last_error.restype = C.c_char_p
        if hasattr(L, "loamx_build_info"):
            L.loamx_build_info.restype = C.c_char_p
        if hasattr(L, "loamx_dist_pack_clouds"):
            L.loamx_dist_pack_clouds.argtypes = [C.c_uint32, C.c_void_p, C.c_void_p, C.c_void_p, C.c_void_p, C.c_uint64, C.c_void_p]
            L.loamx_dist_unpack_clouds_header.argtypes = [C.c_void_p, C.c_uint64, C.c_void_p, C.c_void_p, C.c_void_p, C.c_uint32]
            L.loamx_dist_unpack_clouds_stream.argtypes = [C.c_void_p, C.c_uint64, C.c_uint32, C.c_void_p, C.c_void_p, C.c_void_p]
            L.loamx_dist_gatherv.argtypes = [C.c_void_p, C.c_void_p, C.c_uint32, C.c_int, C.c_void_p, C.c_uint64, C.c_void_p]
        for n in ("loamx_scanreg_create", "loamx_odom_create", "loamx_map_create", "loamx_batch_create",
                  "loamx_batch_stream"):
            if hasattr(L, n):
                getattr(L, n).restype = C.c_void_p
        _lib = L
    return _lib


def _check(rc):
    if rc < 0:
        raise LoamxError(rc, lib().loamx_last_error().decode())
    return rc


def device_count() -> int:
    return int(lib().loamx_device_count())


def pinned_empty(shape, dtype=np.float32):
    import weakref
    L = lib()
    L.loamx_host_alloc.restype = C.c_void_p
    L.loamx_host_alloc.argtypes = [C.c_size_t]
    L.loamx_host_free.argtypes = [C.c_void_p]
    shape = tuple(int(x) for x in (shape if hasattr(shape, "__len__") else (shape,)))
    nbytes = max(int(np.prod(shape)) * np.dtype(dtype).itemsize, 1)
    ptr = L.loamx_host_alloc(nbytes)
    if not ptr:
        raise LoamxError(E_HIP, "loamx_host_alloc failed")
    buf = (C.c_char * nbytes).from_address(ptr)
    weakref.finalize(buf, L.loamx_host_free, C.c_void_p(ptr))
    return np.frombuffer(buf, dtype=dtype, count=int(np.prod(shape))).reshape(shape)


def pinned_copy(a, dtype=np.float32):
    out = pinned_empty(np.shape(a), dtype)
    out[...] = a
    return out


def build_info() -> dict:
    return dict(kv.split("=", 1) for kv in lib().loamx_build_info().decode().split(";") if kv)


def as_points(a) -> np.ndarray:
    a = np.ascontiguousarray(a, dtype=np.float32)
    if a.ndim == 1:
        a = a.reshape(-1, 4)
    assert a.ndim == 2 and a.shape[1] in (4, 8), "points must be (N,4) packed xyzi or (N,8) PCL PointXYZI records"
    return a


def cloud_of(a: np.ndarray) -> Cloud:
    stride = a.shape[1] * 4
    return Cloud(a.ctypes.data if a.size else None, a.shape[0], stride, 12 if stride == 16 else 16, 0)


def to_pcl_layout(a: np.ndarray) -> np.ndarray:
    out = np.zeros((len(a), 8), np.float32)
    out[:, :3] = a[:, :3]
    out[:, 3] = 1.0
    out[:, 4] = a[:, 3]
    return out


def _cfg(struct_t, default_fn, **kw):
    c = struct_t()
    getattr(lib(), default_fn)(C.byref(c))
    for k, v in kw.items():
        assert hasattr(c, k), k
        setattr(c, k, v)
    return c


class Batch:

    def __init__(self, max_sweeps: int, **cfg):
        self._c = _cfg(MapConfig, "loamx_map_default_config", **cfg)
        self.h = C.c_void_p(lib().loamx_batch_create(C.byref(self._c), max_sweeps))
        if not self.h:
            raise LoamxError(E_INVALID, lib().loamx_last_error().decode())
        self.n = 0
        self._keep = []

    def close(self):
        if getattr(self, "h", None):
            lib().loamx_batch_destroy(self.h)
            self.h = None

    __del__ = close

    def set_frozen(self, corner_map, surf_map):
        c, s = as_points(corner_map), as_points(surf_map)
        cc, sc = cloud_of(c), cloud_of(s)
        _check(lib().loamx_batch_set_frozen(self.h, C.byref(cc), C.byref(sc)))

    def set_frozen_device(self, d_corner_ptr: int, n_corner: int, d_surf_ptr: int, n_surf: int):
        _check(lib().loamx_batch_set_frozen_device(self.h, C.c_void_p(d_corner_ptr), n_corner, C.c_void_p(d_surf_ptr), n_surf))

    def stage_frozen_device(self, d_corner_ptr: int, n_corner: int, d_surf_ptr: int, n_surf: int, wait_event: int = 0):
        _check(lib().loamx_batch_stage_frozen_device(self.h, C.c_void_p(d_corner_ptr), n_corner, C.c_void_p(d_surf_ptr), n_surf,
                                                     C.c_void_p(wait_event or None)))

    def stage_frozen(self, corner_map, surf_map):
        cm, sm = as_points(corner_map), as_points(surf_map)
        cc, sc = cloud_of(cm), cloud_of(sm)
        _check(lib().loamx_batch_stage_frozen(self.h, C.byref(cc), C.byref(sc)))

    def swap_frozen(self) -> bool:
        return _check(lib().loamx_batch_swap_frozen(self.h)) == OK

    def upload(self, corner_last, surf_last, guesses, full_res=None):
        n = len(corner_last)
        assert len(surf_last) == n and len(guesses) == n
        cl = [as_points(a) for a in corner_last]
        sl = [as_points(a) for a in surf_last]
        fr = [as_points(a) for a in full_res] if full_res is not None else None
        CA = (Cloud * n)(*[cloud_of(a) for a in cl])
        SA = (Cloud * n)(*[cloud_of(a) for a in sl])
        FA = (Cloud * n)(*[cloud_of(a) for a in fr]) if fr is not None else None
        g = np.ascontiguousarray(guesses, np.float32).reshape(n, 6)
        _check(lib().loamx_batch_upload(self.h, n, CA, SA, FA, g.ctypes.data_as(C.c_void_p)))
        self.n = n
        self._full_sizes = [len(a) for a in fr] if fr is not None else None

    def run(self):
        return _check(lib().loamx_batch_run(self.h))

    def run_async(self):
        _check(lib().loamx_batch_run_async(self.h))

    def sync(self):
        _check(lib().loamx_batch_sync(self.h))

    def download(self):
        poses = np.zeros((self.n, 6), np.float32)
        stats = np.zeros((self.n, 4), np.int32)
        _check(lib().loamx_batch_download(self.h, poses.ctypes.data_as(C.c_void_p), stats.ctypes.data_as(C.c_void_p)))
        return poses, stats

    def download_full_res(self, sweep: int):
        out = np.zeros((self._full_sizes[sweep], 4), np.float32)
        c = cloud_of(out)
        _check(lib().loamx_batch_download_full_res(self.h, sweep, C.byref(c)))
        return out[:c.count]

    def download_ds(self, sweep: int, cap: int = 1 << 17):
        co, so = np.zeros((cap, 4), np.float32), np.zeros((cap, 4), np.float32)
        cc, sc = cloud_of(co), cloud_of(so)
        _check(lib().loamx_batch_download_ds(self.h, sweep, C.byref(cc), C.byref(sc)))
        return co[:cc.count].copy(), so[:sc.count].copy()

    def qr6_probe(self, ata, atb):
        A = np.ascontiguousarray(ata, np.float32).reshape(-1, 36)
        b = np.ascontiguousarray(atb, np.float32).reshape(-1, 6)
        assert len(A) == len(b)
        xc, xs = np.zeros_like(b), np.zeros_like(b)
        _check(lib().loamx_batch_qr6_probe(self.h, A.ctypes.data_as(C.c_void_p), b.ctypes.data_as(C.c_void_p), len(A),
                                           xc.ctypes.data_as(C.c_void_p), xs.ctypes.data_as(C.c_void_p)))
        return xc, xs

    def xrec_stress(self, pairs: int = 64, rounds: int = 20000):
        out = (C.c_uint64 * 4)()
        _check(lib().loamx_batch_xrec_stress(self.h, pairs, rounds, out))
        return dict(accepted=int(out[0]), torn=int(out[1]), inconsistent=int(out[2]), timed_out=int(out[3]))

    def knn_probe(self, which: int, queries_xyz):
        q = np.ascontiguousarray(np.asarray(queries_xyz, np.float32)[:, :3])
        idx = np.zeros((len(q), 5), np.uint32)
        d2 = np.zeros((len(q), 5), np.float32)
        _check(lib().loamx_batch_knn_probe(self.h, which, q.ctypes.data_as(C.c_void_p), len(q), idx.ctypes.data_as(C.c_void_p),
                                           d2.ctypes.data_as(C.c_void_p)))
        return idx, d2

    def set_timing(self, on: bool):
        _check(lib().loamx_batch_set_timing(self.h, 1 if on else 0))

    def timing(self):
        ms = (C.c_float * 4)()
        cnt = (C.c_uint64 * 4)()
        _check(lib().loamx_batch_get_timing(self.h, ms, cnt))
        return dict(run_ms=ms[0], residual_ms=ms[1], residual_launches=int(cnt[0]), query_iterations=int(cnt[1]),
                    queries=int(cnt[2]))

    @property
    def stream(self) -> int:
        return int(lib().loamx_batch_stream(self.h) or 0)


class TransformMaintenance:

    def __init__(self):
        lib().loamx_tm_create.restype = C.c_void_p
        self.h = C.c_void_p(lib().loamx_tm_create())

    def close(self):
        if getattr(self, "h", None):
            lib().loamx_tm_destroy(self.h)
            self.h = None

    __del__ = close

    def update_odometry(self, transform_sum):
        t = np.ascontiguousarray(transform_sum, np.float32)
        _check(lib().loamx_tm_update_odometry(self.h, t.ctypes.data_as(C.c_void_p)))

    def update_mapping_transform(self, aft_mapped, bef_mapped):
        a, b = np.ascontiguousarray(aft_mapped, np.float32), np.ascontiguousarray(bef_mapped, np.float32)
        _check(lib().loamx_tm_update_mapping_transform(self.h, a.ctypes.data_as(C.c_void_p), b.ctypes.data_as(C.c_void_p)))

    def associate_to_map(self):
        _check(lib().loamx_tm_associate_to_map(self.h))
        out = np.zeros(6, np.float32)
        _check(lib().loamx_tm_get_mapped(self.h, out.ctypes.data_as(C.c_void_p)))
        return out


def wire_pose_to_quat(rot_xyz):
    r = np.ascontiguousarray(rot_xyz, np.float32)
    q = np.zeros(4, np.float64)
    _check(lib().loamx_wire_pose_to_quat(r.ctypes.data_as(C.c_void_p), q.ctypes.data_as(C.c_void_p)))
    return q


def wire_quat_to_pose(quat_xyzw):
    q = np.ascontiguousarray(quat_xyzw, np.float64)
    r = np.zeros(3, np.float32)
    _check(lib().loamx_wire_quat_to_pose(q.ctypes.data_as(C.c_void_p), r.ctypes.data_as(C.c_void_p)))
    return r


class MultiScanMapper(C.Structure):
    _fields_ = [("lower_bound_deg", C.c_float), ("upper_bound_deg", C.c_float), ("n_scan_rings", C.c_uint32)]


class ScanRegistration:
    NAMES = ("sharp", "less_sharp", "flat", "less_flat")

    def __init__(self, **cfg):
        self._c = _cfg(ScanRegConfig, "loamx_scanreg_default_config", **cfg)
        self.h = C.c_void_p(lib().loamx_scanreg_create(C.byref(self._c)))
        if not self.h:
            raise LoamxError(E_INVALID, lib().loamx_last_error().decode())

    def close(self):
        if getattr(self, "h", None):
            lib().loamx_scanreg_destroy(self.h)
            self.h = None

    __del__ = close

    def configure(self, **cfg):
        for k, v in cfg.items():
            assert hasattr(self._c, k), k
            setattr(self._c, k, v)
        _check(lib().loamx_scanreg_configure(self.h, C.byref(self._c)))

    def process(self, points, ring_sizes, pcl_layout=False):
        pts = as_points(points)
        rs = np.ascontiguousarray(ring_sizes, np.uint32)
        n = len(pts)
        width = 8 if pcl_layout else 4
        key = (max(n, 1), width)
        if getattr(self, "_out_key", None) != key:
            self._outs = [np.zeros(key, np.float32) for _ in range(4)]
            self._out_key = key
        outs = self._outs
        cl = [cloud_of(o) for o in outs]
        cin = cloud_of(pts)
        _check(lib().loamx_scanreg_process(self.h, C.byref(cin), rs.ctypes.data_as(C.c_void_p), len(rs), C.byref(cl[0]),
                                           C.byref(cl[1]), C.byref(cl[2]), C.byref(cl[3])))
        res = {name: outs[k][:cl[k].count].copy() for k, name in enumerate(self.NAMES)}
        res["full"] = pts
        return res

    def process_linked(self, points, ring_sizes):
        pts = as_points(points)
        rs = np.ascontiguousarray(ring_sizes, np.uint32)
        cin = cloud_of(pts)
        self._linked_n = len(pts)
        return _check(lib().loamx_scanreg_process_linked(self.h, C.byref(cin), rs.ctypes.data_as(C.c_void_p), len(rs)))

    def update_imu(self, stamp, roll, pitch, yaw, acc):
        a = np.ascontiguousarray(acc, np.float32)
        _check(lib().loamx_scanreg_update_imu(self.h, C.c_double(stamp), C.c_float(roll), C.c_float(pitch), C.c_float(yaw),
                                              a.ctypes.data_as(C.c_void_p)))

    def set_time(self, t):
        _check(lib().loamx_scanreg_set_time(self.h, C.c_double(t)))

    def imu_trans(self):
        out = np.zeros(12, np.float32)
        _check(lib().loamx_scanreg_get_imu_trans(self.h, out.ctypes.data_as(C.c_void_p)))
        return out

    def process_raw(self, raw_xyz, sensor="VLP-16", mapper=None):
        raw = np.ascontiguousarray(raw_xyz, np.float32).reshape(-1, 3)
        m = MultiScanMapper()
        if mapper is None:
            _check(lib().loamx_multiscan_mapper_preset(sensor.encode(), C.byref(m)))
        else:
            m.lower_bound_deg, m.upper_bound_deg, m.n_scan_rings = float(mapper[0]), float(mapper[1]), int(mapper[2])
        n = len(raw)
        outs = [np.zeros((max(n, 1), 4), np.float32) for _ in range(5)]
        cl = [cloud_of(o) for o in outs]
        rs = np.zeros(max(int(m.n_scan_rings), 1), np.uint32)
        _check(lib().loamx_scanreg_process_raw(self.h, C.byref(m), raw.ctypes.data_as(C.c_void_p), n, 12, C.byref(cl[4]),
                                               rs.ctypes.data_as(C.c_void_p), C.byref(cl[0]), C.byref(cl[1]), C.byref(cl[2]),
                                               C.byref(cl[3])))
        res = {name: outs[k][:cl[k].count].copy() for k, name in enumerate(self.NAMES)}
        res["full"] = outs[4][:cl[4].count].copy()
        res["ring_sizes"] = rs.astype(np.int32)
        return res


class LaserOdometry:

    def __init__(self, **cfg):
        self._c = _cfg(OdomConfig, "loamx_odom_default_config", **cfg)
        self.h = C.c_void_p(lib().loamx_odom_create(C.byref(self._c)))
        if not self.h:
            raise LoamxError(E_INVALID, lib().loamx_last_error().decode())
        self._sizes = (0, 0)

    def close(self):
        if getattr(self, "h", None):
            lib().loamx_odom_destroy(self.h)
            self.h = None

    __del__ = close

    def update_imu(self, t12):
        t = np.ascontiguousarray(t12, np.float32)
        _check(lib().loamx_odom_update_imu(self.h, t.ctypes.data_as(C.c_void_p)))

    def process(self, feats):
        arrs = [as_points(feats[n]) for n in ("sharp", "less_sharp", "flat", "less_flat")]
        cl = [cloud_of(a) for a in arrs]
        rc = _check(lib().loamx_odom_process(self.h, C.byref(cl[0]), C.byref(cl[1]), C.byref(cl[2]), C.byref(cl[3])))
        self._sizes = (len(arrs[1]), len(arrs[3]))
        return rc

    def process_linked(self, scanreg):
        rc = _check(lib().loamx_odom_process_linked(self.h, scanreg.h))
        self._sizes = (scanreg._linked_n, scanreg._linked_n)
        return rc

    def link_wait(self):
        return _check(lib().loamx_odom_link_wait(self.h))

    def _t(self, fn):
        t = np.zeros(6, np.float32)
        _check(fn(self.h, t.ctypes.data_as(C.c_void_p)))
        return t

    @property
    def transform(self):
        return self._t(lib().loamx_odom_get_transform)

    @property
    def transform_sum(self):
        return self._t(lib().loamx_odom_get_transform_sum)

    def set_transform(self, t6):
        t = np.ascontiguousarray(t6, np.float32)
        _check(lib().loamx_odom_set_transform(self.h, t.ctypes.data_as(C.c_void_p)))

    def set_transform_sum(self, t6):
        t = np.ascontiguousarray(t6, np.float32)
        _check(lib().loamx_odom_set_transform_sum(self.h, t.ctypes.data_as(C.c_void_p)))

    def last_clouds(self):
        c = np.zeros((max(self._sizes[0], 1), 4), np.float32)
        s = np.zeros((max(self._sizes[1], 1), 4), np.float32)
        cc, sc = cloud_of(c), cloud_of(s)
        _check(lib().loamx_odom_get_last_clouds(self.h, C.byref(cc), C.byref(sc)))
        return c[:cc.count].copy(), s[:sc.count].copy()

    def transform_to_end(self, cloud):
        a = as_points(cloud).copy()
        c = cloud_of(a)
        _check(lib().loamx_odom_transform_to_end(self.h, C.byref(c)))
        return a

    def stats(self):
        s = (C.c_int * 4)()
        _check(lib().loamx_odom_get_stats(self.h, s))
        return dict(iterations=s[0], sel=s[1], frame=s[2], degenerate=s[3])


class LaserMapping:

    def __init__(self, **cfg):
        self._c = _cfg(MapConfig, "loamx_map_default_config", **cfg)
        self.h = C.c_void_p(lib().loamx_map_create(C.byref(self._c)))
        if not self.h:
            raise LoamxError(E_INVALID, lib().loamx_last_error().decode())

    def close(self):
        if getattr(self, "h", None):
            lib().loamx_map_destroy(self.h)
            self.h = None

    __del__ = close

    def update_odometry(self, t6):
        t = np.ascontiguousarray(t6, np.float32)
        _check(lib().loamx_map_update_odometry(self.h, t.ctypes.data_as(C.c_void_p)))

    def update_imu(self, stamp, roll, pitch):
        _check(lib().loamx_map_update_imu(self.h, C.c_double(stamp), C.c_float(roll), C.c_float(pitch)))

    def set_time(self, t):
        _check(lib().loamx_map_set_time(self.h, C.c_double(t)))

    def process(self, corner_last, surf_last, full_res=None, inplace=False):
        c, s = as_points(corner_last), as_points(surf_last)
        cc, sc = cloud_of(c), cloud_of(s)
        if full_res is not None:
            f = as_points(full_res) if inplace else as_points(full_res).copy()
            fc = cloud_of(f)
            rc = _check(lib().loamx_map_process(self.h, C.byref(cc), C.byref(sc), C.byref(fc)))
            return rc, f
        rc = _check(lib().loamx_map_process(self.h, C.byref(cc), C.byref(sc), None))
        return rc, None

    def process_linked(self, odometry, full_out=None):
        if full_out is None:
            return _check(lib().loamx_map_process_linked(self.h, odometry.h, None)), None
        fc = cloud_of(full_out)
        rc = _check(lib().loamx_map_process_linked(self.h, odometry.h, C.byref(fc)))
        return rc, full_out[:fc.count]

    def speculation(self):
        c = (C.c_uint64 * 2)()
        _check(lib().loamx_map_get_speculation(self.h, c))
        return int(c[0]), int(c[1])

    def insert(self, corner_last, surf_last, pose6):
        c, s = as_points(corner_last), as_points(surf_last)
        cc, sc = cloud_of(c), cloud_of(s)
        p = np.ascontiguousarray(pose6, np.float32)
        assert p.shape == (6,)
        return _check(lib().loamx_map_insert(self.h, C.byref(cc), C.byref(sc), p.ctypes.data_as(C.c_void_p)))

    def transform(self, which="aft"):
        t = np.zeros(6, np.float32)
        _check(lib().loamx_map_get_transform(self.h, ("aft", "bef", "tobe", "sum").index(which), t.ctypes.data_as(C.c_void_p)))
        return t

    def set_transform(self, which, t6):
        t = np.ascontiguousarray(t6, np.float32)
        _check(lib().loamx_map_set_transform(self.h, ("aft", "bef", "tobe", "sum").index(which), t.ctypes.data_as(C.c_void_p)))

    def set_timing(self, on: bool):
        _check(lib().loamx_map_set_timing(self.h, 1 if on else 0))

    def timing(self):
        ms = (C.c_float * 4)()
        cnt = (C.c_uint64 * 4)()
        _check(lib().loamx_map_get_timing(self.h, ms, cnt))
        return dict(run_ms=ms[0], residual_ms=ms[1], residual_launches=int(cnt[0]), query_iterations=int(cnt[1]), queries=int(cnt[2]))

    def has_fresh_map(self):
        return bool(lib().loamx_map_has_fresh_map(self.h))

    def _get(self, fn, *args, cap=1 << 16):
        while True:
            out = np.zeros((cap, 4), np.float32)
            c = cloud_of(out)
            rc = fn(self.h, *args, C.byref(c))
            if rc == E_CAPACITY:
                cap = int(c.count) + 16
                continue
            _check(rc)
            return out[:c.count].copy()

    def save_snapshot(self, path: str):
        _check(lib().loamx_map_save_snapshot(self.h, path.encode()))

    def load_snapshot(self, path: str):
        _check(lib().loamx_map_load_snapshot(self.h, path.encode()))

    def surround(self):
        return self._get(lib().loamx_map_get_surround)

    def cubes(self, which):
        return self._get(lib().loamx_map_get_cubes, 0 if which == "corner" else 1)

    def load_cubes(self, corner, surf):
        c, s = as_points(corner), as_points(surf)
        cc, sc = cloud_of(c), cloud_of(s)
        _check(lib().loamx_map_load_cubes(self.h, C.byref(cc), C.byref(sc)))

    def stats(self):
        s = (C.c_int * 8)()
        _check(lib().loamx_map_get_stats(self.h, s))
        keys = ("iterations", "sel", "corner_ds", "surf_ds", "corner_from_map", "surf_from_map", "degenerate", "optimized")
        return dict(zip(keys, (int(v) for v in s)))


class Pipeline:

    def __init__(self, n_streams: int, scanreg=None, odom=None, mapping=None):
        self._f = _cfg(ScanRegConfig, "loamx_scanreg_default_config", **(scanreg or {}))
        self._o = _cfg(OdomConfig, "loamx_odom_default_config", **(odom or {}))
        self._m = _cfg(MapConfig, "loamx_map_default_config", **(mapping or {}))
        L = lib()
        L.loamx_pipeline_create.restype = C.c_void_p
        L.loamx_pipeline_stream.restype = C.c_void_p
        self.h = C.c_void_p(L.loamx_pipeline_create(C.byref(self._f), C.byref(self._o), C.byref(self._m), n_streams))
        if not self.h:
            raise LoamxError(E_INVALID, L.loamx_last_error().decode())
        self.n_streams = n_streams
        self._sizes = None

    def close(self):
        if getattr(self, "h", None):
            lib().loamx_pipeline_destroy(self.h)
            self.h = None

    __del__ = close

    def set_frozen(self, corner_map, surf_map):
        c, s = as_points(corner_map), as_points(surf_map)
        cc, sc = cloud_of(c), cloud_of(s)
        _check(lib().loamx_pipeline_set_frozen(self.h, C.byref(cc), C.byref(sc)))

    def set_frozen_device(self, d_corner_ptr, n_corner, d_surf_ptr, n_surf):
        _check(lib().loamx_pipeline_set_frozen_device(self.h, C.c_void_p(d_corner_ptr), n_corner, C.c_void_p(d_surf_ptr), n_surf))

    def stage_frozen_device(self, d_corner_ptr, n_corner, d_surf_ptr, n_surf, wait_event: int = 0):
        _check(lib().loamx_pipeline_stage_frozen_device(self.h, C.c_void_p(d_corner_ptr), n_corner, C.c_void_p(d_surf_ptr), n_surf,
                                                        C.c_void_p(wait_event or None)))

    def stage_frozen(self, corner_map, surf_map):
        cm, sm = as_points(corner_map), as_points(surf_map)
        cc, sc = cloud_of(cm), cloud_of(sm)
        _check(lib().loamx_pipeline_stage_frozen(self.h, C.byref(cc), C.byref(sc)))

    def swap_frozen(self) -> bool:
        return _check(lib().loamx_pipeline_swap_frozen(self.h)) == OK

    def set_state(self, stream, transform=None, transform_sum=None, bef=None, aft=None):
        def p(a):
            if a is None:
                return None
            a = np.ascontiguousarray(a, np.float32)
            keep.append(a)
            return a.ctypes.data_as(C.c_void_p)
        keep = []
        _check(lib().loamx_pipeline_set_state(self.h, stream, p(transform), p(transform_sum), p(bef), p(aft)))

    def upload(self, sweeps):
        n_steps = len(sweeps)
        ns = self.n_streams
        pts, rings = [], []
        for t in range(n_steps):
            assert len(sweeps[t]) == ns
            for s in range(ns):
                pts.append(as_points(sweeps[t][s][0]))
                rings.append(np.ascontiguousarray(sweeps[t][s][1], np.uint32))
        CA = (Cloud * len(pts))(*[cloud_of(a) for a in pts])
        RP = (C.c_void_p * len(pts))(*[r.ctypes.data for r in rings])
        NR = (C.c_uint32 * len(pts))(*[len(r) for r in rings])
        _check(lib().loamx_pipeline_upload(self.h, n_steps, CA, RP, NR))
        self._sizes = [len(a) for a in pts]

    def stage_step(self, t: int, sweeps_t):
        ns = self.n_streams
        assert len(sweeps_t) == ns
        pts = [as_points(sweeps_t[s][0]) for s in range(ns)]
        rings = [np.ascontiguousarray(sweeps_t[s][1], np.uint32) for s in range(ns)]
        CA = (Cloud * ns)(*[cloud_of(a) for a in pts])
        RP = (C.c_void_p * ns)(*[r.ctypes.data for r in rings])
        NR = (C.c_uint32 * ns)(*[len(r) for r in rings])
        _check(lib().loamx_pipeline_stage_step(self.h, t, CA, RP, NR))
        if not hasattr(self, "_staged"):
            self._staged = {}
        self._staged[t % 8] = (pts, rings, CA, RP, NR)

    def stage_step_raw(self, t: int, raws, sensor="VLP-16", mapper=None, scan_times=None):
        ns = self.n_streams
        assert len(raws) == ns
        arrs = [np.ascontiguousarray(r, np.float32).reshape(-1, 3) for r in raws]
        m = MultiScanMapper()
        if mapper is None:
            _check(lib().loamx_multiscan_mapper_preset(sensor.encode(), C.byref(m)))
        else:
            m.lower_bound_deg, m.upper_bound_deg, m.n_scan_rings = float(mapper[0]), float(mapper[1]), int(mapper[2])
        PP = (C.c_void_p * ns)(*[a.ctypes.data if len(a) else None for a in arrs])
        CN = (C.c_uint32 * ns)(*[len(a) for a in arrs])
        st = (C.c_double * ns)(*[float(x) for x in scan_times]) if scan_times is not None else None
        _check(lib().loamx_pipeline_stage_step_raw(self.h, t, PP, CN, 12, C.byref(m), st))
        if not hasattr(self, "_staged"):
            self._staged = {}
        self._staged[t % 8] = (arrs, PP, CN, st)

    def update_imu(self, stream: int, stamp, roll, pitch, yaw, acc):
        a = np.ascontiguousarray(acc, np.float32)
        _check(lib().loamx_pipeline_update_imu(self.h, stream, C.c_double(stamp), C.c_float(roll), C.c_float(pitch), C.c_float(yaw),
                                               a.ctypes.data_as(C.c_void_p)))

    def enable_async_downloads(self):
        _check(lib().loamx_pipeline_enable_async_downloads(self.h))

    def download_step_async(self, outs):
        CA = (Cloud * len(outs))(*[cloud_of(a) for a in outs])
        _check(lib().loamx_pipeline_download_step_async(self.h, CA, len(outs)))
        self._dl_keep = (outs, CA)
        return [int(CA[k].count) for k in range(len(outs))]

    def wait_downloads(self):
        _check(lib().loamx_pipeline_wait_downloads(self.h))

    def download_counts(self):
        c = (C.c_uint64 * 2)()
        _check(lib().loamx_pipeline_download_counts(self.h, c))
        return int(c[0]), int(c[1])

    def step(self, t: int):
        return _check(lib().loamx_pipeline_step(self.h, t))

    def get(self, stream: int):
        tr, ts, aft = (np.zeros(6, np.float32) for _ in range(3))
        st = (C.c_int * 8)()
        _check(lib().loamx_pipeline_get(self.h, stream, tr.ctypes.data_as(C.c_void_p), ts.ctypes.data_as(C.c_void_p),
                                        aft.ctypes.data_as(C.c_void_p), st))
        keys = ("odom_iterations", "odom_sel", "map_iterations", "map_sel", "corner_ds", "surf_ds", "degenerate", "mapped")
        return tr, ts, aft, dict(zip(keys, (int(v) for v in st)))

    def download_full_res(self, slot: int, n: int):
        out = np.zeros((n, 4), np.float32)
        c = cloud_of(out)
        _check(lib().loamx_pipeline_download_full_res(self.h, slot, C.byref(c)))
        return out[:c.count]

    def last_clouds(self, stream: int, capacity: int):
        c, s = np.zeros((max(capacity, 1), 4), np.float32), np.zeros((max(capacity, 1), 4), np.float32)
        cc, sc = cloud_of(c), cloud_of(s)
        _check(lib().loamx_pipeline_download_last_clouds(self.h, stream, C.byref(cc), C.byref(sc)))
        return c[:cc.count].copy(), s[:sc.count].copy()

    def set_lookahead(self, on: bool):
        _check(lib().loamx_pipeline_set_lookahead(self.h, 1 if on else 0))

    def lookahead_depth(self) -> int:
        return int(lib().loamx_pipeline_lookahead_depth(self.h))

    def drain_lookahead(self):
        last = C.c_int(-1)
        _check(lib().loamx_pipeline_drain_lookahead(self.h, C.byref(last)))
        return int(last.value)

    def set_timing(self, on, per_launch: bool = True):
        _check(lib().loamx_pipeline_set_timing(self.h, (1 if per_launch else 2) if on else 0))

    def timing(self):
        ms = (C.c_float * 4)()
        rms = (C.c_float * 4)()
        cnt = (C.c_uint64 * 4)()
        _check(lib().loamx_pipeline_get_timing(self.h, ms, rms, cnt))
        return dict(features_ms=ms[0], odometry_ms=ms[1], registration_ms=ms[2], step_ms=ms[3], reg_run_ms=rms[0],
                    residual_ms=rms[1], residual_launches=int(cnt[0]), query_iterations=int(cnt[1]), queries=int(cnt[2]))

    def odom_launch_timing(self):
        ms = (C.c_double * 4)()
        cnt = (C.c_uint64 * 7)()
        _check(lib().loamx_pipeline_get_odom_launch_timing(self.h, ms, cnt))
        return dict(lm_ms=ms[0], lm_noop_ms=ms[1], corr_ms=ms[2], corr_noop_ms=ms[3], lm_launches=int(cnt[0]), lm_noop_launches=int(cnt[1]),
                    lm_iterations=int(cnt[2]), corr_launches=int(cnt[3]), corr_noop_launches=int(cnt[4]), lm_bytes=int(cnt[5]),
                    corr_features=int(cnt[6]))

    @property
    def stream(self) -> int:
        return int(lib().loamx_pipeline_stream(self.h) or 0)


def dist_shard_of(rank: int, world: int, batch: int):
    b, e = C.c_uint32(0), C.c_uint32(0)
    _check(lib().loamx_dist_shard_of(rank, world, batch, C.byref(b), C.byref(e)))
    return int(b.value), int(e.value)


def dist_pack_results(poses6, iters_flags, n_pad: int) -> np.ndarray:
    p = np.ascontiguousarray(poses6, np.float32).reshape(-1, 6)
    f = np.ascontiguousarray(iters_flags, np.int32).reshape(len(p), 2) if iters_flags is not None else None
    out = np.zeros((n_pad, 8), np.float32)
    _check(lib().loamx_dist_pack_results(p.ctypes.data_as(C.c_void_p), f.ctypes.data_as(C.c_void_p) if f is not None else None, len(p), n_pad,
                                         out.ctypes.data_as(C.c_void_p)))
    return out


def dist_unpack_results(recv, counts, n_pad: int):
    r = np.ascontiguousarray(recv, np.float32)
    c = np.ascontiguousarray(counts, np.uint32)
    tot = int(c.sum())
    pa, fa = np.zeros((max(tot, 1), 6), np.float32), np.zeros((max(tot, 1), 2), np.int32)
    _check(lib().loamx_dist_unpack_results(r.ctypes.data_as(C.c_void_p), c.ctypes.data_as(C.c_void_p), len(c), n_pad, pa.ctypes.data_as(C.c_void_p),
                                           fa.ctypes.data_as(C.c_void_p)))
    return pa[:tot], fa[:tot]


def dist_pack_clouds(corners, surfs, poses6) -> np.ndarray:
    cs = [as_points(c) for c in corners]
    ss = [as_points(c) for c in surfs]
    n = len(cs)
    assert len(ss) == n
    p = np.ascontiguousarray(poses6, np.float32).reshape(n, 6) if n else np.zeros((0, 6), np.float32)
    CA = Cloud * max(n, 1)
    ca, sa = CA(*[cloud_of(c) for c in cs]), CA(*[cloud_of(c) for c in ss])
    nw = C.c_uint64(0)
    _check(lib().loamx_dist_pack_clouds(n, C.addressof(ca), C.addressof(sa), p.ctypes.data, None, 0, C.addressof(nw)))
    out = np.zeros(int(nw.value), np.uint32)
    _check(lib().loamx_dist_pack_clouds(n, C.addressof(ca), C.addressof(sa), p.ctypes.data, out.ctypes.data, len(out), C.addressof(nw)))
    return out


def dist_unpack_clouds(words):
    w = np.ascontiguousarray(words, np.uint32)
    ns = C.c_uint32(0)
    _check(lib().loamx_dist_unpack_clouds_header(w.ctypes.data, len(w), C.addressof(ns), None, None, 0))
    n = int(ns.value)
    nc, nsf = np.zeros(max(n, 1), np.uint32), np.zeros(max(n, 1), np.uint32)
    _check(lib().loamx_dist_unpack_clouds_header(w.ctypes.data, len(w), C.addressof(ns), nc.ctypes.data, nsf.ctypes.data, max(n, 1)))
    out = []
    for s in range(n):
        pose = np.zeros(6, np.float32)
        co, so = np.zeros((max(int(nc[s]), 1), 4), np.float32), np.zeros((max(int(nsf[s]), 1), 4), np.float32)
        cc, sc = cloud_of(co), cloud_of(so)
        _check(lib().loamx_dist_unpack_clouds_stream(w.ctypes.data, len(w), s, pose.ctypes.data, C.addressof(cc), C.addressof(sc)))
        out.append((pose, co[:cc.count].copy(), so[:sc.count].copy()))
    return out


def dist_split_messages(words, counts):
    out, o = [], 0
    for c in counts:
        c = int(c)
        out.append(np.ascontiguousarray(words[o:o + c]) if c else None)
        o += c
    return out


class Dist:
    ID_BYTES = 128

    @staticmethod
    def unique_id() -> bytes:
        buf = (C.c_ubyte * Dist.ID_BYTES)()
        _check(lib().loamx_dist_get_unique_id(buf))
        return bytes(buf)

    def __init__(self, unique_id: bytes, rank: int, world_size: int, device: int = 0):
        assert len(unique_id) == self.ID_BYTES
        L = lib()
        L.loamx_dist_create.restype = C.c_void_p
        L.loamx_dist_stream.restype = C.c_void_p
        buf = (C.c_ubyte * self.ID_BYTES).from_buffer_copy(unique_id)
        self.h = C.c_void_p(L.loamx_dist_create(buf, rank, world_size, device))
        if not self.h:
            raise LoamxError(E_INVALID, L.loamx_last_error().decode())
        self.rank, self.world = rank, world_size

    def close(self):
        if getattr(self, "h", None):
            lib().loamx_dist_destroy(self.h)
            self.h = None

    __del__ = close

    def shard(self, batch: int):
        b, e = C.c_uint32(), C.c_uint32()
        _check(lib().loamx_dist_shard(self.h, batch, C.byref(b), C.byref(e)))
        return int(b.value), int(e.value)

    def broadcast_map(self, d_corner_ptr: int, n_corner: int, d_surf_ptr: int, n_surf: int, root: int = 0, wait_event: int = 0) -> int:
        ev = C.c_void_p()
        _check(lib().loamx_dist_broadcast_map(self.h, C.c_void_p(d_corner_ptr), n_corner, C.c_void_p(d_surf_ptr), n_surf, root,
                                              C.c_void_p(wait_event or None), C.byref(ev)))
        return int(ev.value or 0)

    def allgather_results(self, poses6, iters_flags=None, batch=None):
        p = np.ascontiguousarray(poses6, np.float32).reshape(-1, 6)
        n = len(p)
        f = np.ascontiguousarray(iters_flags, np.int32).reshape(n, 2) if iters_flags is not None else None
        cnt = np.zeros(self.world, np.uint32)
        _check(lib().loamx_dist_allgather_counts(self.h, n, cnt.ctypes.data_as(C.c_void_p)))
        cap = int(cnt.sum())
        pa = np.zeros((max(cap, 1), 6), np.float32)
        fa = np.zeros((max(cap, 1), 2), np.int32)
        _check(lib().loamx_dist_allgather_results_cap(self.h, p.ctypes.data_as(C.c_void_p), f.ctypes.data_as(C.c_void_p) if f is not None else None,
                                                      n, pa.ctypes.data_as(C.c_void_p), fa.ctypes.data_as(C.c_void_p), cap, cnt.ctypes.data_as(C.c_void_p)))
        tot = int(cnt.sum())
        if batch is not None and int(batch) != cap:
            raise ValueError(f"allgather_results: batch = {batch} but the ranks hold {cap} records")
        return pa[:tot], fa[:tot], cnt

    def allgather_counts(self, n: int) -> np.ndarray:
        cnt = np.zeros(self.world, np.uint32)
        _check(lib().loamx_dist_allgather_counts(self.h, int(n), cnt.ctypes.data_as(C.c_void_p)))
        return cnt

    def gatherv(self, words, root: int = 0):
        w = np.ascontiguousarray(words if words is not None else np.zeros(0, np.uint32), np.uint32)
        cnt = np.zeros(self.world, np.uint32)
        _check(lib().loamx_dist_allgather_counts(self.h, len(w), cnt.ctypes.data_as(C.c_void_p)))
        tot = int(cnt.sum())
        recv = np.zeros(max(tot, 1), np.uint32) if self.rank == root else None
        _check(lib().loamx_dist_gatherv(self.h, w.ctypes.data, len(w), root, recv.ctypes.data if recv is not None else None,
                                        tot if recv is not None else 0, cnt.ctypes.data))
        return (dist_split_messages(recv[:tot], cnt) if recv is not None else None), cnt

    def comm_count(self) -> int:
        return int(lib().loamx_dist_comm_count(self.h))

    def barrier(self):
        _check(lib().loamx_dist_barrier(self.h))

    @property
    def stream(self) -> int:
        return int(lib().loamx_dist_stream(self.h) or 0)
```

Baseline: 16400.

## Split odometry correspondence search into sub-wave lane groups handling multiple features

```diff
diff --git a/include/loamx.h b/include/loamx.h
--- a/include/loamx.h
+++ b/include/loamx.h
@@ -91,6 +91,8 @@
 int loamx_odom_get_last_clouds(loamx_odom* h, loamx_cloud* last_corner, loamx_cloud* last_surf);
 int loamx_odom_transform_to_end(loamx_odom* h, loamx_cloud* cloud);
 int loamx_odom_get_stats(loamx_odom* h, int stats[4]);
+int loamx_odom_corr_probe(loamx_odom* h, int lanes, const loamx_cloud* sharp, const loamx_cloud* flat, uint32_t n_rep, const float* transforms6,
+                          const uint32_t* counts2, const int* done, int* ind3, uint8_t* path);
 
 int loamx_scanreg_process_linked(loamx_scanreg* h, const loamx_cloud* cloud, const uint32_t* ring_size, uint32_t n_rings);
 int loamx_odom_process_linked(loamx_odom* h, loamx_scanreg* sr);
diff --git a/loam_velodyne_amd/csrc/api_odom.hip b/loam_velodyne_amd/csrc/api_odom.hip
--- a/loam_velodyne_amd/csrc/api_odom.hip
+++ b/loam_velodyne_amd/csrc/api_odom.hip
@@ -96,4 +96,17 @@
   });
 }
 
+int loamx_odom_corr_probe(loamx_odom* h, int lanes, const loamx_cloud* sharp, const loamx_cloud* flat, uint32_t n_rep, const float* transforms6,
+                          const uint32_t* counts2, const int* done, int* ind3, uint8_t* path) {
+  return guard([&]() {
+    LX_REQUIRE(h && sharp && flat, "NULL argument");
+    check_cloud(sharp, false);
+    check_cloud(flat, false);
+    std::vector<float4> s(sharp->count + 1), f(flat->count + 1);
+    pack_cloud(sharp, s.data());
+    pack_cloud(flat, f.data());
+    return h->od.corr_probe(lanes, s.data(), sharp->count, f.data(), flat->count, n_rep, transforms6, counts2, done, ind3, path);
+  });
 }
+
+}
diff --git a/loam_velodyne_amd/csrc/odometry.hip b/loam_velodyne_amd/csrc/odometry.hip
--- a/loam_velodyne_amd/csrc/odometry.hip
+++ b/loam_velodyne_amd/csrc/odometry.hip
@@ -34,30 +34,68 @@
   return dx * dx + dy * dy + dz * dz;
 }
 
-__device__ inline void wave_argmin(float& d, int& j, int& order) {
-#pragma unroll
-  for (int off = 32; off > 0; off >>= 1) {
-    const float od = __shfl_xor(d, off, 64);
-    const int oj = __shfl_xor(j, off, 64);
-    const int oo = __shfl_xor(order, off, 64);
-    if (od < d || (od == d && oo < order)) { d = od; j = oj; order = oo; }
-  }
-}
-
-__device__ inline int nn1_shells(const GridDesc& g, const float4* __restrict__ sorted, const uint32_t* __restrict__ cell_start, float qx,
-                                 float qy, float qz, int lane, int L0, float best, int best_id) {
+template <int G>
+__device__ inline unsigned long long grp_bits(unsigned long long m, int lane) {
+  if constexpr (G == 64) return m;
+  else return (m >> (lane & ~(G - 1))) & ((1ull << G) - 1ull);
+}
+template <int OFF>
+__device__ inline int bfly_partner(int v) {
+  if constexpr (OFF == 1) return __builtin_amdgcn_mov_dpp(v, 0xB1, 0xF, 0xF, false);
+  else if constexpr (OFF == 2) return __builtin_amdgcn_mov_dpp(v, 0x4E, 0xF, 0xF, false);
+  else if constexpr (OFF == 4) return __builtin_amdgcn_mov_dpp(v, 0x141, 0xF, 0xF, false);
+  else if constexpr (OFF == 8) return __builtin_amdgcn_mov_dpp(v, 0x140, 0xF, 0xF, false);
+  else if constexpr (OFF == 16) return __builtin_amdgcn_ds_swizzle(v, 0x401F);
+  else return __shfl_xor(v, 32, 64);
+}
+template <int OFF>
+__device__ inline void argmin_step(float& d, int& j, int& order, int& carry) {
+  const float od = __int_as_float(bfly_partner<OFF>(__float_as_int(d)));
+  const int oj = bfly_partner<OFF>(j), oo = bfly_partner<OFF>(order), oc = bfly_partner<OFF>(carry);
+  if (od < d || (od == d && oo < order)) { d = od; j = oj; order = oo; carry = oc; }
+}
+template <int G>
+__device__ inline void grp_argmin(float& d, int& j, int& order, int& carry) {
+  argmin_step<1>(d, j, order, carry);
+  argmin_step<2>(d, j, order, carry);
+  if constexpr (G > 4) argmin_step<4>(d, j, order, carry);
+  if constexpr (G > 8) argmin_step<8>(d, j, order, carry);
+  if constexpr (G > 16) argmin_step<16>(d, j, order, carry);
+  if constexpr (G > 32) argmin_step<32>(d, j, order, carry);
+}
+template <int G>
+__device__ inline int grp_min(int v) {
+  v = min(v, bfly_partner<1>(v));
+  v = min(v, bfly_partner<2>(v));
+  if constexpr (G > 4) v = min(v, bfly_partner<4>(v));
+  if constexpr (G > 8) v = min(v, bfly_partner<8>(v));
+  if constexpr (G > 16) v = min(v, bfly_partner<16>(v));
+  if constexpr (G > 32) v = min(v, bfly_partner<32>(v));
+  return v;
+}
+template <int G>
+__device__ inline void grp_argmin(float& d, int& j, int& order) {
+  int c = 0;
+  grp_argmin<G>(d, j, order, c);
+}
+
+template <int G>
+__device__ __forceinline__ int nn1_shells(const GridDesc& g, const float4* __restrict__ sorted, const uint32_t* __restrict__ cell_start, float qx,
+                                 float qy, float qz, int lane, bool need, int L0, float best, int best_id) {
+  const int gl = lane & (G - 1);
   float lbest = best;
   uint32_t lid = best_id >= 0 ? (uint32_t)best_id : 0xffffffffu;
   const float h = 1.0f / g.inv_h;
   const float fx = (qx - g.ox) * g.inv_h, fy = (qy - g.oy) * g.inv_h, fz = (qz - g.oz) * g.inv_h;
   const int cx = (int)floorf(fx), cy = (int)floorf(fy), cz = (int)floorf(fz);
-  for (int L = L0;; L++) {
+  bool done = !need;
+  for (int L = L0; __ballot(!done); L++) {
     const int side = 2 * L + 1, nrows = side * side;
-    for (int r0 = 0; r0 < nrows; r0 += 64) {
+    for (int r0 = 0; r0 < nrows; r0 += G) {
       uint32_t b0 = 0, e0 = 0, b1 = 0, e1 = 0;
       {
-        const int rr = r0 + lane;
-        if (rr < nrows) {
+        const int rr = r0 + gl;
+        if (!done && rr < nrows) {
           const int dz = rr / side - L, dy = rr % side - L;
           const int z = cz + dz, y = cy + dy;
           if (z >= 0 && z < g.nz && y >= 0 && y < g.ny) {
@@ -83,19 +121,22 @@
           }
         }
       }
-      unsigned long long todo = __ballot(e0 > b0 || e1 > b1);
-      while (todo) {
-        const int src = __builtin_ctzll(todo);
+      unsigned long long todo = grp_bits<G>(__ballot(e0 > b0 || e1 > b1), lane);
+      while (__ballot(todo != 0ull)) {
+        const bool have = todo != 0ull;
+        const int src = have ? __builtin_ctzll(todo) : 0;
         todo &= todo - 1;
-        const uint32_t rb0 = __shfl(b0, src, 64), re0 = __shfl(e0, src, 64), rb1 = __shfl(b1, src, 64), re1 = __shfl(e1, src, 64);
-        for (int part = 0; part < 2; part++) {
-          const uint32_t beg = part ? rb1 : rb0, end = part ? re1 : re0;
-          for (uint32_t k = beg + lane; k < end; k += 64) {
-            const float4 p = sorted[k];
-            const float dx = qx - p.x, dy2 = qy - p.y, dz2 = qz - p.z;
-            const float d2 = dx * dx + dy2 * dy2 + dz2 * dz2;
-            const uint32_t id = __float_as_uint(p.w) & OD_IDX_MASK;
-            if (d2 < lbest || (d2 == lbest && lid != 0xffffffffu && id < lid)) { lbest = d2; lid = id; }
+        const uint32_t rb0 = __shfl(b0, src, G), re0 = __shfl(e0, src, G), rb1 = __shfl(b1, src, G), re1 = __shfl(e1, src, G);
+        if (have) {
+          for (int part = 0; part < 2; part++) {
+            const uint32_t beg = part ? rb1 : rb0, end = part ? re1 : re0;
+            for (uint32_t k = beg + gl; k < end; k += G) {
+              const float4 p = sorted[k];
+              const float dx = qx - p.x, dy2 = qy - p.y, dz2 = qz - p.z;
+              const float d2 = dx * dx + dy2 * dy2 + dz2 * dz2;
+              const uint32_t id = __float_as_uint(p.w) & OD_IDX_MASK;
+              if (d2 < lbest || (d2 == lbest && lid != 0xffffffffu && id < lid)) { lbest = d2; lid = id; }
+            }
           }
         }
       }
@@ -103,11 +144,12 @@
     float d = lbest;
     int j = (int)lid, o_ = (int)lid;
     if (lid == 0xffffffffu) { j = -1; o_ = 0x7fffffff; }
-    wave_argmin(d, j, o_);
-    if (j >= 0 && d < 25.0f) { best = d; best_id = j; }
-    const float cover = (float)L * h;
-    if (best <= cover * cover) break;
-    if (cover * cover >= 25.0f) break;
+    grp_argmin<G>(d, j, o_);
+    if (!done) {
+      if (j >= 0 && d < 25.0f) { best = d; best_id = j; }
+      const float cover = (float)L * h;
+      if (best <= cover * cover || cover * cover >= 25.0f) done = true;
+    }
   }
   return best_id;
 }
@@ -116,72 +158,96 @@
 #else
 #define OD_CORR_ATTR
 #endif
+#ifndef OD_BLK_CACHE
+#define OD_BLK_CACHE 2
+#endif
+template <int G>
+struct CorrShape {
+  static constexpr int NF = 64 / G;
+  static constexpr int U = G == 64 ? 4 : 8;
+  static constexpr int TRIP = G * U;
+  static constexpr int NC = OD_BLK_CACHE * 64 / G < U ? OD_BLK_CACHE * 64 / G : U;
+  static constexpr int NT = 64 / G;
+};
 struct Block27 {
   uint32_t E[9], O[9];
   uint32_t total;
 };
-__device__ inline void block27_build(const GridDesc& g, const uint32_t* __restrict__ cell_start, float qx, float qy, float qz, int lane, Block27& B) {
+template <int G>
+__device__ __forceinline__ void block27_build(const GridDesc& g, const uint32_t* __restrict__ cell_start, float qx, float qy, float qz, int lane, Block27& B) {
+  constexpr int NV = (18 + G - 1) / G;
+  const int gl = lane & (G - 1);
   const float fx = (qx - g.ox) * g.inv_h, fy = (qy - g.oy) * g.inv_h, fz = (qz - g.oz) * g.inv_h;
   const int cx = (int)floorf(fx), cy = (int)floorf(fy), cz = (int)floorf(fz);
-  uint32_t v = 0u;
-  {
-    const int r = lane >> 1, z = cz + r / 3 - 1, y = cy + r % 3 - 1;
-    if (lane < 18 && z >= 0 && z < g.nz && y >= 0 && y < g.ny) {
-      int xx = (lane & 1) ? cx + 2 : cx - 1;
+  uint32_t v[NV];
+#pragma unroll
+  for (int k = 0; k < NV; k++) {
+    const int b = gl + G * k, r = b >> 1, z = cz + r / 3 - 1, y = cy + r % 3 - 1;
+    v[k] = 0u;
+    if (b < 18 && z >= 0 && z < g.nz && y >= 0 && y < g.ny) {
+      int xx = (b & 1) ? cx + 2 : cx - 1;
       xx = xx < 0 ? 0 : (xx > g.nx ? g.nx : xx);
-      v = cell_start[((uint32_t)z * g.ny + y) * g.nx + xx];
+      v[k] = cell_start[((uint32_t)z * g.ny + y) * g.nx + xx];
     }
   }
   uint32_t acc = 0;
 #pragma unroll
   for (int r = 0; r < 9; r++) {
-    const uint32_t b = (uint32_t)__shfl((int)v, 2 * r, 64), e = (uint32_t)__shfl((int)v, 2 * r + 1, 64);
+    const uint32_t b = (uint32_t)__shfl((int)v[(2 * r) / G], (2 * r) % G, G), e = (uint32_t)__shfl((int)v[(2 * r + 1) / G], (2 * r + 1) % G, G);
     B.O[r] = b - acc;
     acc += e > b ? e - b : 0u;
     B.E[r] = acc;
   }
   B.total = acc;
 }
-#ifndef OD_BLK_CACHE
-#define OD_BLK_CACHE 2
-#endif
-struct Block27First { float4 p[OD_BLK_CACHE > 0 ? OD_BLK_CACHE : 1]; };
-template <bool LOAD_FIRST, class F>
-__device__ inline void block27_scan(const Block27& B, const float4* __restrict__ sorted, int lane, Block27First& first, F&& visit) {
-  for (uint32_t c0 = (uint32_t)lane; c0 < B.total; c0 += 4 * 64) {
-    const bool first_trip = c0 == (uint32_t)lane;
-    uint32_t pos[4];
-    float4 p[4];
-#pragma unroll
-    for (int u = 0; u < 4; u++) {
-      const uint32_t cc = c0 + 64u * u;
+template <int G>
+struct Block27First { float4 p[CorrShape<G>::NC > 0 ? CorrShape<G>::NC : 1]; };
+template <int G, bool LOAD_FIRST, class F>
+__device__ __forceinline__ void block27_scan(const Block27& B, const float4* __restrict__ sorted, int lane, Block27First<G>& first, F&& visit) {
+  constexpr int U = CorrShape<G>::U, NC = CorrShape<G>::NC;
+  const uint32_t gl = (uint32_t)(lane & (G - 1));
+  auto positions = [&](uint32_t c0, uint32_t (&pos)[U]) {
+#pragma unroll
+    for (int u = 0; u < U; u++) {
+      const uint32_t cc = c0 + (uint32_t)G * u;
       uint32_t o = B.O[8];
 #pragma unroll
       for (int k = 7; k >= 0; k--) o = cc < B.E[k] ? B.O[k] : o;
       pos[u] = cc < B.total ? cc + o : B.O[0];
     }
-    if (LOAD_FIRST || !first_trip) {
-#pragma unroll
-      for (int u = 0; u < 4; u++) p[u] = sorted[pos[u]];
-      if (LOAD_FIRST && first_trip) {
-#pragma unroll
-        for (int u = 0; u < OD_BLK_CACHE; u++) first.p[u] = p[u];
-      }
-    } else {
-#pragma unroll
-      for (int u = OD_BLK_CACHE; u < 4; u++) p[u] = sorted[pos[u]];
-#pragma unroll
-      for (int u = 0; u < OD_BLK_CACHE; u++) p[u] = first.p[u];
-    }
-#pragma unroll
-    for (int u = 0; u < 4; u++) visit(p[u], (c0 + 64u * u) < B.total);
-  }
-}
-__device__ inline int nn1_block(const GridDesc& g, const Block27& B, const float4* __restrict__ sorted, const uint32_t* __restrict__ cell_start,
-                                float qx, float qy, float qz, int lane, uint32_t& w_out, Block27First& first) {
+  };
+  uint32_t c0 = gl;
+  if (c0 >= B.total) return;
+  {
+    uint32_t pos[U];
+    float4 p[U];
+    positions(c0, pos);
+#pragma unroll
+    for (int u = LOAD_FIRST ? 0 : NC; u < U; u++) p[u] = sorted[pos[u]];
+#pragma unroll
+    for (int u = 0; u < NC; u++) {
+      if (LOAD_FIRST) first.p[u] = p[u];
+      else p[u] = first.p[u];
+    }
+#pragma unroll
+    for (int u = 0; u < U; u++) visit(p[u], (c0 + (uint32_t)G * u) < B.total);
+  }
+  for (c0 += CorrShape<G>::TRIP; c0 < B.total; c0 += CorrShape<G>::TRIP) {
+    uint32_t pos[U];
+    float4 p[U];
+    positions(c0, pos);
+#pragma unroll
+    for (int u = 0; u < U; u++) p[u] = sorted[pos[u]];
+#pragma unroll
+    for (int u = 0; u < U; u++) visit(p[u], (c0 + (uint32_t)G * u) < B.total);
+  }
+}
+template <int G>
+__device__ __forceinline__ int nn1_block(const GridDesc& g, const Block27& B, const float4* __restrict__ sorted, const uint32_t* __restrict__ cell_start,
+                                float qx, float qy, float qz, int lane, uint32_t& w_out, bool& shells, Block27First<G>& first) {
   float lbest = 25.0f;
   uint32_t lw = 0xffffffffu;
-  block27_scan<true>(B, sorted, lane, first, [&](const float4& p, bool valid) {
+  block27_scan<G, true>(B, sorted, lane, first, [&](const float4& p, bool valid) {
     const float dx = qx - p.x, dy2 = qy - p.y, dz2 = qz - p.z;
     const float d2 = dx * dx + dy2 * dy2 + dz2 * dz2;
     const uint32_t w = __float_as_uint(p.w);
@@ -190,45 +256,48 @@
   float d = lbest;
   int j = lw == 0xffffffffu ? -1 : (int)(lw & OD_IDX_MASK), o_ = lw == 0xffffffffu ? 0x7fffffff : (int)(lw & OD_IDX_MASK);
   int ring = (int)(lw >> 24);
-  {
-#pragma unroll
-    for (int off = 32; off > 0; off >>= 1) {
-      const float od = __shfl_xor(d, off, 64);
-      const int oj = __shfl_xor(j, off, 64), oo = __shfl_xor(o_, off, 64), orr = __shfl_xor(ring, off, 64);
-      if (od < d || (od == d && oo < o_)) { d = od; j = oj; o_ = oo; ring = orr; }
-    }
-  }
+  grp_argmin<G>(d, j, o_, ring);
   const float h = 1.0f / g.inv_h;
-  if (j >= 0 && d < 25.0f && d <= h * h) { w_out = ((uint32_t)ring << 24) | (uint32_t)j; return j; }
-  const int id = nn1_shells(g, sorted, cell_start, qx, qy, qz, lane, 2, (j >= 0 && d < 25.0f) ? d : 25.0f, (j >= 0 && d < 25.0f) ? j : -1);
+  const bool hit = j >= 0 && d < 25.0f && d <= h * h;
+  shells = !hit;
+  const int id = nn1_shells<G>(g, sorted, cell_start, qx, qy, qz, lane, !hit, 2, (j >= 0 && d < 25.0f) ? d : 25.0f, (j >= 0 && d < 25.0f) ? j : -1);
+  if (hit) { w_out = ((uint32_t)ring << 24) | (uint32_t)j; return j; }
   w_out = id == j ? (((uint32_t)ring << 24) | (uint32_t)j) : (0xff000000u | (uint32_t)(id < 0 ? 0 : id));
   return id;
 }
 
 constexpr int OD_RF_N = 320;
+constexpr uint8_t OD_PATH_BLOCK = 1, OD_PATH_WALK = 2, OD_PATH_SHELLS = 4;
 #ifdef LOAMX_PROF_CORR
 __device__ unsigned long long g_corr_ts[3][16];
-#define OC_TS(k) do { if (blockIdx.y == 0 && lane == 0 && ts_slot >= 0) g_corr_ts[ts_slot][k] = wall_clock64(); } while (0)
+#define OC_TS(k) do { if (blockIdx.y == 0 && gl == 0 && ts_slot >= 0) g_corr_ts[ts_slot][k] = wall_clock64(); } while (0)
 #else
 #define OC_TS(k) do { } while (0)
 #endif
-__global__ __launch_bounds__(256) OD_CORR_ATTR void k_odom_corr_grid(OdomProblem* __restrict__ probs, OdomParams P, uint32_t* __restrict__ patch_dst, uint4 patch) {
+template <int G>
+__global__ __launch_bounds__(256) OD_CORR_ATTR void k_odom_corr_grid(OdomProblem* __restrict__ probs, OdomParams P, uint32_t* __restrict__ patch_dst, uint4 patch,
+                                                                      uint8_t* __restrict__ paths, uint32_t path_stride) {
+  using S = CorrShape<G>;
   if (patch_dst && blockIdx.x == 0 && blockIdx.y == 0 && threadIdx.x == 0) { patch_dst[0] = patch.x; patch_dst[1] = patch.y; patch_dst[2] = patch.z; }
   OdomProblem& pb = probs[blockIdx.y];
   if (pb.done) return;
-  const int lane = threadIdx.x & 63, wid = threadIdx.x >> 6;
+  const int lane = threadIdx.x & 63, gl = lane & (G - 1), wid = threadIdx.x >> 6;
   const int nSharp = (int)pb.n_sharp, nFlat = (int)pb.n_flat;
   int f;
+  bool live;
   {
     const int x = (int)(blockIdx.x % 8), j = (int)(blockIdx.x / 8);
     const int sS = (int)((long long)x * nSharp / 8), nS = (int)((long long)(x + 1) * nSharp / 8) - sS;
     const int sF = (int)((long long)x * nFlat / 8), nF = (int)((long long)(x + 1) * nFlat / 8) - sF;
-    const int fl = 4 * j + wid;
-    if (fl >= nS + nF) return;
+    const int fl0 = 4 * S::NF * j + S::NF * wid;
+    if (fl0 >= nS + nF) return;
+    int fl = fl0 + lane / G;
+    live = fl < nS + nF;
+    if (!live) fl = fl0;
     f = fl < nS ? sS + fl : nSharp + sF + (fl - nS);
   }
 #ifdef LOAMX_PROF_CORR
-  const int ts_slot = f == nSharp / 2 ? 0 : f == nSharp + nFlat / 2 ? 1 : f == nSharp + nFlat - 1 ? 2 : -1;
+  const int ts_slot = !live ? -1 : f == nSharp / 2 ? 0 : f == nSharp + nFlat / 2 ? 1 : f == nSharp + nFlat - 1 ? 2 : -1;
 #endif
   OC_TS(0);
   float T[6];
@@ -238,11 +307,10 @@
   const float4 pi = corner ? pb.sharp[f] : pb.flat[f - nSharp];
   const uint32_t* __restrict__ tbl = corner ? pb.rf_corner : pb.rf_surf;
   const int e0 = max((int)pi.w - 8, 0);
-  uint32_t tv = 0u, unordered_epoch = 0u;
-  if (tbl) {
-    if (e0 + lane < OD_RF_N - 1) tv = tbl[e0 + lane];
-    unordered_epoch = tbl[OD_RF_N - 1];
-  }
+  uint32_t tv[S::NT], unordered_epoch = 0u;
+#pragma unroll
+  for (int k = 0; k < S::NT; k++) tv[k] = tbl && e0 + G * k + gl < OD_RF_N - 1 ? tbl[e0 + G * k + gl] : 0u;
+  if (tbl) unordered_epoch = tbl[OD_RF_N - 1];
   float x, y, z;
   transform_to_start(T, P.scan_period, pi, x, y, z);
   const GridDescB gd = corner ? *pb.lc_desc : *pb.ls_desc;
@@ -250,105 +318,122 @@
   const uint32_t* __restrict__ cell_start = pb.cell_table + gd.cell_base;
   OC_TS(1);
   Block27 B;
-  block27_build(gd.g, cell_start, x, y, z, lane, B);
+  block27_build<G>(gd.g, cell_start, x, y, z, lane, B);
   OC_TS(2);
   uint32_t wbest = 0u;
-  Block27First first;
-  const int closest = nn1_block(gd.g, B, sorted, cell_start, x, y, z, lane, wbest, first);
+  bool shells = false;
+  Block27First<G> first;
+  const int closest = nn1_block<G>(gd.g, B, sorted, cell_start, x, y, z, lane, wbest, shells, first);
   OC_TS(3);
-  if (closest < 0) {
-    if (lane == 0) { pb.ind[5 * f] = -1; pb.ind[5 * f + 1] = -1; pb.ind[5 * f + 2] = -1; }
-    return;
-  }
+  const bool has = closest >= 0;
   const float4* last = corner ? pb.last_corner : pb.last_surf;
   const int nLast = corner ? (int)pb.n_last_corner : (int)pb.n_last_surf;
   const int nCur = corner ? nSharp : nFlat;
   const int bound = nCur < nLast ? nCur : nLast;
-  const int cscan = (wbest >> 24) != 255u ? (int)(wbest >> 24) : (int)last[closest].w;
+  const int cscan = !has ? 0 : (wbest >> 24) != 255u ? (int)(wbest >> 24) : (int)last[closest].w;
   float d2 = 25.f, d3 = 25.f;
   int j2 = -1, j3 = -1, o2 = 0x7fffffff, o3 = 0x7fffffff;
   auto better = [](float d, int order, float dbest, int obest) { return d < dbest || (d == dbest && obest != 0x7fffffff && order < obest); };
 
   bool via_block = false;
-  if (tbl && unordered_epoch != pb.rf_epoch && cscan < 255 && B.total > 0u) {
-    const unsigned long long valid = __ballot(e0 + lane < OD_RF_N - 1 && (tv >> 24) == pb.rf_epoch);
-    auto first_from = [&](int ring) -> int {
+  {
+    unsigned long long valid = 0ull;
+#pragma unroll
+    for (int k = 0; k < S::NT; k++) valid |= grp_bits<G>(__ballot(e0 + G * k + gl < OD_RF_N - 1 && (tv[k] >> 24) == pb.rf_epoch), lane) << (G * k);
+    auto first_entry = [&](int ring) -> int {
       const int k = ring - e0;
-      if (k >= 64) return nLast;
+      if (k >= 64) return -1;
       const unsigned long long m = k <= 0 ? valid : (valid >> k) << k;
-      if (!m) return nLast;
-      const int w = (int)((uint32_t)__shfl((int)tv, __builtin_ctzll(m), 64) & OD_IDX_MASK);
+      return m ? __builtin_ctzll(m) : -1;
+    };
+    auto entry = [&](int i) -> uint32_t {
+      uint32_t s = tv[0];
+#pragma unroll
+      for (int k = 1; k < S::NT; k++) s = i / G == k ? tv[k] : s;
+      return (uint32_t)__shfl((int)s, i % G, G);
+    };
+    const int ilo = first_entry(cscan - 2), ihi = first_entry(cscan + 3);
+    const uint32_t tlo = entry(ilo < 0 ? 0 : ilo), thi = entry(ihi < 0 ? 0 : ihi);
+    auto first_from = [&](int i, uint32_t t) -> int {
+      if (i < 0) return nLast;
+      const int w = (int)(t & OD_IDX_MASK);
       return w < nLast ? w : nLast;
     };
-    if (cscan - 2 >= e0 || e0 == 0) {
-      const int wlo = min(first_from(cscan - 2), closest);
-      const int whi = closest + 1 < bound ? max(min(bound, first_from(cscan + 3)), closest + 1) : closest + 1;
+    if (has && tbl && unordered_epoch != pb.rf_epoch && cscan < 255 && B.total > 0u && (cscan - 2 >= e0 || e0 == 0)) {
+      const int wlo = min(first_from(ilo, tlo), closest);
+      const int whi = closest + 1 < bound ? max(min(bound, first_from(ihi, thi)), closest + 1) : closest + 1;
       const unsigned walk = (unsigned)(closest - wlo) + (unsigned)(whi - (closest + 1));
-      via_block = walk > B.total + 128u;
+      via_block = walk > B.total + (unsigned)S::TRIP / 2u;
     }
   }
   OC_TS(4);
-  if (via_block) {
-    block27_scan<false>(B, sorted, lane, first, [&](const float4& p, bool ok) {
-      const uint32_t w = __float_as_uint(p.w);
-      const int j = (int)(w & OD_IDX_MASK), ring = (int)(w >> 24);
-      const float d = sqd(p, x, y, z);
-      if (ok && j > closest && j < bound && ring <= cscan + 2) {
-        const int order = j - (closest + 1);
-        if (corner) {
-          if (ring > cscan && better(d, order, d2, o2)) { d2 = d; j2 = j; o2 = order; }
-        } else {
-          if (ring <= cscan) { if (better(d, order, d2, o2)) { d2 = d; j2 = j; o2 = order; } }
-          else { if (better(d, order, d3, o3)) { d3 = d; j3 = j; o3 = order; } }
-        }
-      } else if (ok && j < closest && ring >= cscan - 2) {
-        const int order = 0x40000000 + (closest - 1 - j);
-        if (corner) {
-          if (ring < cscan && better(d, order, d2, o2)) { d2 = d; j2 = j; o2 = order; }
-        } else {
-          if (ring >= cscan) { if (better(d, order, d2, o2)) { d2 = d; j2 = j; o2 = order; } }
-          else { if (better(d, order, d3, o3)) { d3 = d; j3 = j; o3 = order; } }
-        }
-      }
-    });
-    wave_argmin(d2, j2, o2);
-    if (!corner) wave_argmin(d3, j3, o3);
+  bool flats = __ballot(!corner) != 0ull;
+  if (__ballot(via_block)) {
+    if (via_block) {
+      block27_scan<G, false>(B, sorted, lane, first, [&](const float4& p, bool ok) {
+        const uint32_t w = __float_as_uint(p.w);
+        const int j = (int)(w & OD_IDX_MASK), ring = (int)(w >> 24);
+        const float d = sqd(p, x, y, z);
+        if (ok && j > closest && j < bound && ring <= cscan + 2) {
+          const int order = j - (closest + 1);
+          if (corner) {
+            if (ring > cscan && better(d, order, d2, o2)) { d2 = d; j2 = j; o2 = order; }
+          } else {
+            if (ring <= cscan) { if (better(d, order, d2, o2)) { d2 = d; j2 = j; o2 = order; } }
+            else { if (better(d, order, d3, o3)) { d3 = d; j3 = j; o3 = order; } }
+          }
+        } else if (ok && j < closest && ring >= cscan - 2) {
+          const int order = 0x40000000 + (closest - 1 - j);
+          if (corner) {
+            if (ring < cscan && better(d, order, d2, o2)) { d2 = d; j2 = j; o2 = order; }
+          } else {
+            if (ring >= cscan) { if (better(d, order, d2, o2)) { d2 = d; j2 = j; o2 = order; } }
+            else { if (better(d, order, d3, o3)) { d3 = d; j3 = j; o3 = order; } }
+          }
+        }
+      });
+    }
+    grp_argmin<G>(d2, j2, o2);
+    if (flats) grp_argmin<G>(d3, j3, o3);
     const float h = 1.0f / gd.g.inv_h, h2 = h * h;
-    via_block = d2 < h2 && (corner || d3 < h2);
+    via_block = via_block && d2 < h2 && (corner || d3 < h2);
     if (!via_block) { d2 = d3 = 25.f; j2 = j3 = -1; o2 = o3 = 0x7fffffff; }
   }
   OC_TS(5);
-  if (!via_block) {
+  const bool walked = has && !via_block;
+  if (__ballot(walked)) {
     int baseF = closest + 1, baseB = closest - 1;
-    bool stopF = baseF >= bound, stopB = baseB < 0;
-    while (!stopF || !stopB) {
-      float4 qf[4], qb[4];
-      if (!stopF) {
-#pragma unroll
-        for (int u = 0; u < 4; u++) {
-          const int j = baseF + 64 * u + lane;
-          qf[u] = j < bound ? last[j] : make_float4(0.f, 0.f, 0.f, 0.f);
-        }
-      }
-      if (!stopB) {
-#pragma unroll
-        for (int u = 0; u < 4; u++) {
-          const int j = baseB - 64 * u - lane;
-          qb[u] = j >= 0 ? last[j] : make_float4(0.f, 0.f, 0.f, 0.f);
-        }
-      }
-      if (!stopF) {
-        bool stop = false;
-#pragma unroll
-        for (int u = 0; u < 4; u++) {
-          if (stop) continue;
-          const int j = baseF + 64 * u + lane;
-          const bool in = j < bound;
-          const int ring = (int)qf[u].w;
-          const bool brk = in && ((double)ring > (double)cscan + 2.5);
-          const unsigned long long mb = __ballot(brk);
-          const int fb = mb ? __builtin_ctzll(mb) : 64;
-          if (in && lane < fb) {
+    bool stopF = !walked || baseF >= bound, stopB = !walked || baseB < 0;
+    while (__ballot(!stopF || !stopB)) {
+      float4 qf[S::U], qb[S::U];
+      const bool anyF = __ballot(!stopF) != 0ull, anyB = __ballot(!stopB) != 0ull;
+      if (anyF) {
+#pragma unroll
+        for (int u = 0; u < S::U; u++) {
+          const int j = baseF + G * u + gl;
+          qf[u] = !stopF && j < bound ? last[j] : make_float4(0.f, 0.f, 0.f, 0.f);
+        }
+      }
+      if (anyB) {
+#pragma unroll
+        for (int u = 0; u < S::U; u++) {
+          const int j = baseB - G * u - gl;
+          qb[u] = !stopB && j >= 0 ? last[j] : make_float4(0.f, 0.f, 0.f, 0.f);
+        }
+      }
+      if (anyF) {
+        int jb = 0x7fffffff;
+#pragma unroll
+        for (int u = S::U - 1; u >= 0; u--) {
+          const int j = baseF + G * u + gl;
+          if (!stopF && j < bound && (int)qf[u].w > cscan + 2) jb = j;
+        }
+        jb = grp_min<G>(jb);
+#pragma unroll
+        for (int u = 0; u < S::U; u++) {
+          const int j = baseF + G * u + gl;
+          if (!stopF && j < bound && j < jb) {
+            const int ring = (int)qf[u].w;
             const float d = sqd(qf[u], x, y, z);
             const int order = j - (closest + 1);
             if (corner) {
@@ -358,23 +443,23 @@
               else { if (better(d, order, d3, o3)) { d3 = d; j3 = j; o3 = order; } }
             }
           }
-          if (mb) stop = true;
-        }
-        baseF += 256;
-        stopF = stop || baseF >= bound;
-      }
-      if (!stopB) {
-        bool stop = false;
-#pragma unroll
-        for (int u = 0; u < 4; u++) {
-          if (stop) continue;
-          const int j = baseB - 64 * u - lane;
-          const bool in = j >= 0;
-          const int ring = (int)qb[u].w;
-          const bool brk = in && ((double)ring < (double)cscan - 2.5);
-          const unsigned long long mb = __ballot(brk);
-          const int fb = mb ? __builtin_ctzll(mb) : 64;
-          if (in && lane < fb) {
+        }
+        baseF += S::TRIP;
+        stopF = stopF || jb != 0x7fffffff || baseF >= bound;
+      }
+      if (anyB) {
+        int jb = -1;
+#pragma unroll
+        for (int u = S::U - 1; u >= 0; u--) {
+          const int j = baseB - G * u - gl;
+          if (!stopB && j >= 0 && (int)qb[u].w < cscan - 2) jb = j;
+        }
+        jb = -grp_min<G>(-jb);
+#pragma unroll
+        for (int u = 0; u < S::U; u++) {
+          const int j = baseB - G * u - gl;
+          if (!stopB && j >= 0 && j > jb) {
+            const int ring = (int)qb[u].w;
             const float d = sqd(qb[u], x, y, z);
             const int order = 0x40000000 + (closest - 1 - j);
             if (corner) {
@@ -384,29 +469,32 @@
               else { if (better(d, order, d3, o3)) { d3 = d; j3 = j; o3 = order; } }
             }
           }
-          if (mb) stop = true;
-        }
-        baseB -= 256;
-        stopB = stop || baseB < 0;
-      }
-    }
-    wave_argmin(d2, j2, o2);
-    if (!corner) wave_argmin(d3, j3, o3);
+        }
+        baseB -= S::TRIP;
+        stopB = stopB || jb >= 0 || baseB < 0;
+      }
+    }
+    grp_argmin<G>(d2, j2, o2);
+    if (flats) grp_argmin<G>(d3, j3, o3);
   }
   OC_TS(6);
-  if (lane == 0) {
-    pb.ind[5 * f] = closest;
-    pb.ind[5 * f + 1] = j2;
-    pb.ind[5 * f + 2] = corner ? -1 : j3;
+  if (live && gl == 0) {
+    pb.ind[5 * f] = has ? closest : -1;
+    pb.ind[5 * f + 1] = has ? j2 : -1;
+    pb.ind[5 * f + 2] = has && !corner ? j3 : -1;
+    if (paths) paths[(size_t)blockIdx.y * path_stride + f] = (uint8_t)((has ? (via_block ? OD_PATH_BLOCK : OD_PATH_WALK) : 0) | (shells ? OD_PATH_SHELLS : 0));
   }
 #ifdef LOAMX_PROF_CORR
-  if (blockIdx.y == 0 && lane == 0 && ts_slot >= 0) {
+  if (blockIdx.y == 0 && gl == 0 && ts_slot >= 0) {
     g_corr_ts[ts_slot][7] = wall_clock64();
     g_corr_ts[ts_slot][8] = (unsigned long long)B.total; g_corr_ts[ts_slot][9] = (unsigned long long)via_block;
     g_corr_ts[ts_slot][10] = (unsigned long long)closest; g_corr_ts[ts_slot][11] = (unsigned long long)cscan;
   }
 #endif
 }
+template __global__ void k_odom_corr_grid<64>(OdomProblem*, OdomParams, uint32_t*, uint4, uint8_t*, uint32_t);
+template __global__ void k_odom_corr_grid<32>(OdomProblem*, OdomParams, uint32_t*, uint4, uint8_t*, uint32_t);
+template __global__ void k_odom_corr_grid<16>(OdomProblem*, OdomParams, uint32_t*, uint4, uint8_t*, uint32_t);
 
 #ifdef LOAMX_PROF_LM
 #define LM_TS(k) do { if (blockIdx.x == 0 && blockIdx.y == 0 && tid == 0 && iter == it_begin + 1) pb.part[OD_PART_TS + (k)] = (double)wall_clock64(); } while (0)
@@ -923,6 +1011,21 @@
   return P;
 }
 
+static void launch_corr_grid(int G, uint32_t max_sharp, uint32_t max_flat, uint32_t na, hipStream_t st, OdomProblem* probs, const OdomParams& P,
+                             uint32_t* patch_dst, uint4 patch, uint8_t* paths, uint32_t path_stride) {
+  const uint32_t per_wg = 4u * 64u / (uint32_t)G;
+  const dim3 grid(8 * (((max_sharp + 7) / 8 + (max_flat + 7) / 8 + per_wg - 1) / per_wg), na);
+  if (G == 64) hipLaunchKernelGGL(k_odom_corr_grid<64>, grid, dim3(256), 0, st, probs, P, patch_dst, patch, paths, path_stride);
+  else if (G == 32) hipLaunchKernelGGL(k_odom_corr_grid<32>, grid, dim3(256), 0, st, probs, P, patch_dst, patch, paths, path_stride);
+  else hipLaunchKernelGGL(k_odom_corr_grid<16>, grid, dim3(256), 0, st, probs, P, patch_dst, patch, paths, path_stride);
+}
+int OdometryBatch::corr_lanes(uint32_t n_feat) {
+  static const int forced = [] { const char* e = getenv("LOAMX_CORR_LANES"); const int v = e ? atoi(e) : 0; return v == 16 || v == 32 || v == 64 ? v : 0; }();
+  if (forced) return forced;
+  (void)n_feat;
+  return 16;
+}
+
 void OdometryBatch::process(const OdomInput* in, int* rc, bool defer_tail) {
   TraceRange trace_range("loamx:odometry");
   LX_HIP(hipSetDevice(device_));
@@ -1075,7 +1178,7 @@
         uint32_t* pd = nullptr;
         uint4 pv = make_uint4(0u, 0u, 0u, 0u);
         if (patch_pending) { patch_pending = false; pd = d_cur_off_.p; pv = make_uint4(h_cur_off_[0], h_cur_off_[1], h_cur_off_[2], 0u); }
-        hipLaunchKernelGGL(k_odom_corr_grid, dim3(8 * (((max_sharp + 7) / 8 + (max_flat + 7) / 8 + 3) / 4), na), dim3(256), 0, st_, prob_.p, params, pd, pv);
+        launch_corr_grid(corr_lanes(na * max_feat), max_sharp, max_flat, na, st_, prob_.p, params, pd, pv, nullptr, 0u);
         if (lk >= 0) LX_HIP(hipEventRecord(lt->ev[3 * lk + 1], st_));
       };
       auto enqueue_lm = [&](int k) {
@@ -1305,6 +1408,71 @@
   return rc;
 }
 
+int OdometryBatch::corr_probe(int lanes, const float4* h_sharp, uint32_t n_sharp, const float4* h_flat, uint32_t n_flat, uint32_t n_rep,
+                              const float* transforms6, const uint32_t* counts2, const int* done, int* ind3, uint8_t* path) {
+  LX_REQUIRE(lanes == 16 || lanes == 32 || lanes == 64, "lanes must be 16, 32 or 64");
+  LX_REQUIRE(n_rep >= 1 && n_rep <= 64, "n_rep must be in [1, 64]");
+  LX_REQUIRE(transforms6 && ind3 && path && (h_sharp || !n_sharp) && (h_flat || !n_flat), "NULL argument");
+  LX_REQUIRE(n_sharp + n_flat <= 32 * OD_THREADS, "more than 8192 sharp+flat features");
+  LX_HIP(hipSetDevice(device_));
+  const uint32_t ns = n_streams(), nf = n_sharp + n_flat;
+  const OdomStream& S = *streams_[0];
+  if (!S.inited || !(S.n_last_corner > 10 && S.n_last_surf > 100)) return LOAMX_SKIPPED;
+  LX_HIP(hipStreamSynchronize(st_));
+  DevBuf<float4> feats;
+  DevBuf<int> ind;
+  DevBuf<uint8_t> codes;
+  DevBuf<OdomProblem> probs;
+  feats.reserve(nf + 1);
+  ind.reserve((size_t)n_rep * 5 * nf + 1);
+  codes.reserve((size_t)n_rep * nf + 1);
+  probs.reserve(n_rep);
+  if (n_sharp) LX_HIP(hipMemcpy(feats.p, h_sharp, sizeof(float4) * n_sharp, hipMemcpyHostToDevice));
+  if (n_flat) LX_HIP(hipMemcpy(feats.p + n_sharp, h_flat, sizeof(float4) * n_flat, hipMemcpyHostToDevice));
+  std::vector<int> h_ind((size_t)n_rep * 5 * nf + 1, -2);
+  std::vector<uint8_t> h_codes((size_t)n_rep * nf + 1, 0xff);
+  LX_HIP(hipMemcpy(ind.p, h_ind.data(), sizeof(int) * h_ind.size(), hipMemcpyHostToDevice));
+  LX_HIP(hipMemcpy(codes.p, h_codes.data(), h_codes.size(), hipMemcpyHostToDevice));
+  std::vector<OdomProblem> hp(n_rep);
+  uint32_t max_sharp = 0, max_flat = 0;
+  for (uint32_t r = 0; r < n_rep; r++) {
+    OdomProblem& pb = hp[r];
+    memset(&pb, 0, sizeof(pb));
+    const uint32_t cs = counts2 ? counts2[2 * r] : n_sharp, cf = counts2 ? counts2[2 * r + 1] : n_flat;
+    LX_REQUIRE(cs <= n_sharp && cf <= n_flat, "counts2 exceeds the clouds");
+    pb.sharp = feats.p; pb.n_sharp = cs;
+    pb.flat = feats.p + n_sharp; pb.n_flat = cf;
+    pb.last_corner = last_.p + h_last_off_[0]; pb.n_last_corner = S.n_last_corner;
+    pb.last_surf = last_.p + h_last_off_[ns]; pb.n_last_surf = S.n_last_surf;
+    pb.sorted = index_.sorted();
+    pb.cell_table = index_.cell_table();
+    pb.lc_desc = index_.desc(0);
+    pb.ls_desc = index_.desc(ns);
+    pb.ind = ind.p + (size_t)r * 5 * nf;
+    memcpy(pb.transform, transforms6 + 6 * r, sizeof(pb.transform));
+    pb.done = done && done[r] ? 1 : 0;
+    pb.rf_corner = rf_.p;
+    pb.rf_surf = rf_.p + (size_t)ns * OD_RF_N;
+    pb.rf_epoch = rf_epoch_;
+    max_sharp = std::max(max_sharp, cs);
+    max_flat = std::max(max_flat, cf);
+  }
+  LX_HIP(hipMemcpy(probs.p, hp.data(), sizeof(OdomProblem) * n_rep, hipMemcpyHostToDevice));
+  if (max_sharp + max_flat) {
+    launch_corr_grid(lanes, max_sharp, max_flat, n_rep, st_, probs.p, params, nullptr, make_uint4(0u, 0u, 0u, 0u), codes.p, nf);
+    LX_HIP(hipGetLastError());
+  }
+  LX_HIP(hipStreamSynchronize(st_));
+  LX_HIP(hipMemcpy(h_ind.data(), ind.p, sizeof(int) * h_ind.size(), hipMemcpyDeviceToHost));
+  LX_HIP(hipMemcpy(h_codes.data(), codes.p, h_codes.size(), hipMemcpyDeviceToHost));
+  for (size_t r = 0; r < n_rep; r++)
+    for (size_t f = 0; f < nf; f++) {
+      for (int k = 0; k < 3; k++) ind3[(r * nf + f) * 3 + k] = h_ind[(r * nf + f) * 5 + k];
+      path[r * nf + f] = h_codes[r * nf + f];
+    }
+  return LOAMX_OK;
+}
+
 int OdometryBatch::process_linked(const float4* const feat[4], const uint32_t n_feat[4], const float4* d_full, uint32_t n_full,
                                   const std::function<void(const float4*&, uint32_t&)>& less_flat_late) {
   LX_REQUIRE(n_streams() == 1, "process_linked is a single-stream entry point");
diff --git a/loam_velodyne_amd/csrc/odometry.hpp b/loam_velodyne_amd/csrc/odometry.hpp
--- a/loam_velodyne_amd/csrc/odometry.hpp
+++ b/loam_velodyne_amd/csrc/odometry.hpp
@@ -108,6 +108,9 @@
   };
   void set_launch_timing(bool on) { launch_timing_.store(on, std::memory_order_relaxed); }
   LaunchTotals launch_totals();
+  int corr_probe(int lanes, const float4* h_sharp, uint32_t n_sharp, const float4* h_flat, uint32_t n_flat, uint32_t n_rep, const float* transforms6,
+                 const uint32_t* counts2, const int* done, int* ind3, uint8_t* path);
+  static int corr_lanes(uint32_t n_feat);
   const float4* d_last_corner(uint32_t s) const { return last_.p + h_last_off_[s]; }
   const float4* d_last_surf(uint32_t s) const { return last_.p + h_last_off_[n_streams() + s]; }
 
diff --git a/loam_velodyne_amd/loamx.py b/loam_velodyne_amd/loamx.py
--- a/loam_velodyne_amd/loamx.py
+++ b/loam_velodyne_amd/loamx.py
@@ -407,6 +407,21 @@
     def link_wait(self):
         return _check(lib().loamx_odom_link_wait(self.h))
 
+    def corr_probe(self, lanes, sharp, flat, transforms, counts=None, done=None):
+        s, f = as_points(sharp), as_points(flat)
+        t = np.ascontiguousarray(np.asarray(transforms, np.float32).reshape(-1, 6))
+        R, nf = len(t), len(s) + len(f)
+        cnt = None if counts is None else np.ascontiguousarray(np.asarray(counts, np.uint32).reshape(R, 2))
+        dn = None if done is None else np.ascontiguousarray(np.asarray(done, np.int32).reshape(R))
+        ind = np.full((R, max(nf, 1), 3), -2, np.int32)
+        path = np.full((R, max(nf, 1)), 0xff, np.uint8)
+        cs, cf = cloud_of(s), cloud_of(f)
+        rc = _check(lib().loamx_odom_corr_probe(self.h, int(lanes), C.byref(cs), C.byref(cf), R, t.ctypes.data_as(C.c_void_p),
+                                                None if cnt is None else cnt.ctypes.data_as(C.c_void_p),
+                                                None if dn is None else dn.ctypes.data_as(C.c_void_p),
+                                                ind.ctypes.data_as(C.c_void_p), path.ctypes.data_as(C.c_void_p)))
+        return rc, ind[:, :nf], path[:, :nf]
+
     def _t(self, fn):
         t = np.zeros(6, np.float32)
         _check(fn(self.h, t.ctypes.data_as(C.c_void_p)))
```

Result: slower. 10750 (median of 2 runs) (-34.4%).
